# gnn-tracking/gnn_tracking

Hardware: AMD Instinct MI355X
Metric: edges_per_sec_fwd_bwd (higher is better)
Workload: dtype bf16

## Files before the change

gnn_tracking_amd/csrc/graph_index.hip:

```cpp
#include "host_util.h"
#include "tile_bf16.h"

namespace gnntrk {

constexpr int kTpb = 256;

constexpr int kSH = 8;
constexpr int kBins = 1 << kSH;
constexpr int kSortTpb = 512;
constexpr int kSortR = 10;
constexpr int kCap = kSortTpb * kSortR;
constexpr int kWin = 4096;
constexpr int kSplitTpb = 1024;
constexpr int kSplitWg = 1;
constexpr int kCountTpb = 1024;
constexpr int kSplitR = 4;
constexpr int kSplitTile = kSplitTpb * kSplitR;
constexpr int kMaxChunks = 512;
#ifndef GNNTRK_GI_HUB_BITMAP_MIN
#define GNNTRK_GI_HUB_BITMAP_MIN 65536
#endif
constexpr int64_t kMaxTable = (int64_t)96 << 20;
constexpr int kScanTpb = 256, kScanItems = 16, kScanTile = kScanTpb * kScanItems;

template <bool kNullable>
__device__ __forceinline__ int64_t gi_clamped(int64_t v, int64_t N, int *bad) {
    if (v < 0 || v >= N) {
        if (!kNullable || bad) atomicAdd(bad, 1);
        v = v < 0 ? 0 : N - 1;
    }
    return v;
}
__device__ __forceinline__ int4 gi_load4(const int32_t *a, int64_t e, int64_t e1) {
    if (e + 4 <= e1) return *reinterpret_cast<const int4 *>(a + e);
    return int4{e < e1 ? a[e] : 0, e + 1 < e1 ? a[e + 1] : 0, e + 2 < e1 ? a[e + 2] : 0, 0};
}

struct KeysCoo {
    const int64_t *src, *tgt;
    int64_t N;
    const uint8_t *label;
    const float *rows;
    int rows_stride;
    __device__ __forceinline__ uint32_t key(int64_t e, int *bad) const { return checked(tgt[e], bad); }
    int vec;
    const int32_t *rank;
    __device__ __forceinline__ uint32_t checked(int64_t v, int *bad) const {
        v = gi_clamped<true>(v, N, bad);
        return rank ? (uint32_t)rank[v] : (uint32_t)v;
    }
    __device__ __forceinline__ void keys4(int64_t e, int64_t e1, uint32_t k[4], int *bad) const {
        if (vec && e + 4 <= e1) {
            const longlong2 a = *reinterpret_cast<const longlong2 *>(tgt + e);
            const longlong2 b = *reinterpret_cast<const longlong2 *>(tgt + e + 2);
            k[0] = checked(a.x, bad);
            k[1] = checked(a.y, bad);
            k[2] = checked(b.x, bad);
            k[3] = checked(b.y, bad);
        } else {
#pragma unroll
            for (int q = 0; q < 4; ++q) k[q] = e + q < e1 ? key(e + q, bad) : 0u;
        }
    }
    struct Raw {
        longlong2 ta, tb, sa, sb;
        uint32_t l4;
    };
    __device__ __forceinline__ void load_raw(int64_t e, int64_t e1, Raw &r) const {
        if (vec && e + 4 <= e1) {
            r.ta = *reinterpret_cast<const longlong2 *>(tgt + e);
            r.tb = *reinterpret_cast<const longlong2 *>(tgt + e + 2);
            r.sa = *reinterpret_cast<const longlong2 *>(src + e);
            r.sb = *reinterpret_cast<const longlong2 *>(src + e + 2);
            r.l4 = label ? *reinterpret_cast<const uint32_t *>(label + e) : 0u;
        } else {
            long long t[4], u[4];
            r.l4 = 0u;
#pragma unroll
            for (int q = 0; q < 4; ++q) {
                const bool in = e + q < e1;
                t[q] = in ? tgt[e + q] : 0;
                u[q] = in ? src[e + q] : 0;
                if (in && label && label[e + q]) r.l4 |= 1u << (8 * q);
            }
            r.ta = longlong2{t[0], t[1]};
            r.tb = longlong2{t[2], t[3]};
            r.sa = longlong2{u[0], u[1]};
            r.sb = longlong2{u[2], u[3]};
        }
    }
    __device__ __forceinline__ void decode(const Raw &r, int64_t e, uint32_t k[4], uint32_t p[4], uint32_t v[4],
                                           int *bad) const {
        k[0] = checked(r.ta.x, nullptr);
        k[1] = checked(r.ta.y, nullptr);
        k[2] = checked(r.tb.x, nullptr);
        k[3] = checked(r.tb.y, nullptr);
        p[0] = checked(r.sa.x, bad);
        p[1] = checked(r.sa.y, bad);
        p[2] = checked(r.sb.x, bad);
        p[3] = checked(r.sb.y, bad);
#pragma unroll
        for (int q = 0; q < 4; ++q) v[q] = (uint32_t)(e + q) | (((r.l4 >> (8 * q)) & 0xffu) ? 0x80000000u : 0u);
    }
    __device__ __forceinline__ f32x4 row_raw(int64_t e) const {
        return *reinterpret_cast<const f32x4 *>(rows + e * rows_stride);
    }
};
struct KeysCoo32 {
    const int32_t *src, *tgt;
    const uint8_t *label;
    const float *rows;
    int rows_stride;
    int vec;
    __device__ __forceinline__ uint32_t key(int64_t e, int *) const { return (uint32_t)tgt[e]; }
    struct Raw {
        int4 t, s;
        uint32_t l4;
    };
    __device__ __forceinline__ void load_raw(int64_t e, int64_t e1, Raw &r) const {
        if (e + 4 <= e1) {
            r.t = *reinterpret_cast<const int4 *>(tgt + e);
            r.s = *reinterpret_cast<const int4 *>(src + e);
            if (!label) {
                r.l4 = 0u;
            } else if (vec) {
                r.l4 = *reinterpret_cast<const uint32_t *>(label + e);
            } else {
                r.l4 = (label[e] ? 1u : 0u) | (label[e + 1] ? 0x100u : 0u) | (label[e + 2] ? 0x10000u : 0u) |
                       (label[e + 3] ? 0x1000000u : 0u);
            }
        } else {
            int t[4], u[4];
            r.l4 = 0u;
#pragma unroll
            for (int q = 0; q < 4; ++q) {
                const bool in = e + q < e1;
                t[q] = in ? tgt[e + q] : 0;
                u[q] = in ? src[e + q] : 0;
                if (in && label && label[e + q]) r.l4 |= 1u << (8 * q);
            }
            r.t = int4{t[0], t[1], t[2], t[3]};
            r.s = int4{u[0], u[1], u[2], u[3]};
        }
    }
    __device__ __forceinline__ void decode(const Raw &r, int64_t e, uint32_t k[4], uint32_t p[4], uint32_t v[4],
                                           int *) const {
        k[0] = (uint32_t)r.t.x;
        k[1] = (uint32_t)r.t.y;
        k[2] = (uint32_t)r.t.z;
        k[3] = (uint32_t)r.t.w;
        p[0] = (uint32_t)r.s.x;
        p[1] = (uint32_t)r.s.y;
        p[2] = (uint32_t)r.s.z;
        p[3] = (uint32_t)r.s.w;
#pragma unroll
        for (int q = 0; q < 4; ++q) v[q] = (uint32_t)(e + q) | (((r.l4 >> (8 * q)) & 0xffu) ? 0x80000000u : 0u);
    }
    __device__ __forceinline__ f32x4 row_raw(int64_t e) const {
        return *reinterpret_cast<const f32x4 *>(rows + e * rows_stride);
    }
};
__device__ __forceinline__ void gi_remap4(const int64_t *__restrict__ src, const int64_t *__restrict__ tgt, int64_t e,
                                          int64_t e1, int64_t N, const int32_t *__restrict__ rank, int vec,
                                          int32_t *__restrict__ src32, int32_t *__restrict__ tgt32,
                                          int *__restrict__ bad, uint32_t kt[4]) {
    if (vec && e + 4 <= e1) {
        typedef int i4_hw __attribute__((ext_vector_type(4)));
        auto ld2 = [](const int64_t *p, long long &a, long long &b) {
            const i4_hw v = __builtin_nontemporal_load(reinterpret_cast<const i4_hw *>(p));
            a = (long long)(((unsigned long long)(uint32_t)v[1] << 32) | (uint32_t)v[0]);
            b = (long long)(((unsigned long long)(uint32_t)v[3] << 32) | (uint32_t)v[2]);
        };
        long long it[4], is[4];
        ld2(tgt + e, it[0], it[1]);
        ld2(tgt + e + 2, it[2], it[3]);
        ld2(src + e, is[0], is[1]);
        ld2(src + e + 2, is[2], is[3]);
#pragma unroll
        for (int q = 0; q < 4; ++q) {
            it[q] = gi_clamped<false>(it[q], N, bad);
            is[q] = gi_clamped<false>(is[q], N, bad);
        }
        const i4_hw ot = {rank[it[0]], rank[it[1]], rank[it[2]], rank[it[3]]};
        const i4_hw os = {rank[is[0]], rank[is[1]], rank[is[2]], rank[is[3]]};
        __builtin_nontemporal_store(ot, reinterpret_cast<i4_hw *>(tgt32 + e));
        __builtin_nontemporal_store(os, reinterpret_cast<i4_hw *>(src32 + e));
#pragma unroll
        for (int q = 0; q < 4; ++q) kt[q] = (uint32_t)ot[q];
    } else {
#pragma unroll
        for (int q = 0; q < 4; ++q) {
            kt[q] = 0u;
            if (e + q < e1) {
                const int t = rank[gi_clamped<false>(tgt[e + q], N, bad)], u = rank[gi_clamped<false>(src[e + q], N, bad)];
                tgt32[e + q] = t;
                src32[e + q] = u;
                kt[q] = (uint32_t)t;
            }
        }
    }
}
struct KeysCsr {
    const int32_t *src;
    __device__ __forceinline__ uint32_t key(int64_t e, int *) const { return (uint32_t)src[e]; }
    __device__ __forceinline__ void keys4(int64_t e, int64_t e1, uint32_t k[4], int *) const {
        const int4 a = gi_load4(src, e, e1);
        k[0] = (uint32_t)a.x;
        k[1] = (uint32_t)a.y;
        k[2] = (uint32_t)a.z;
        k[3] = (uint32_t)a.w;
    }
    struct Raw {
        int4 a;
    };
    __device__ __forceinline__ void load_raw(int64_t e, int64_t e1, Raw &r) const { r.a = gi_load4(src, e, e1); }
    __device__ __forceinline__ void decode(const Raw &r, int64_t e, uint32_t k[4], uint32_t p[4], uint32_t v[4],
                                           int *) const {
        k[0] = (uint32_t)r.a.x;
        k[1] = (uint32_t)r.a.y;
        k[2] = (uint32_t)r.a.z;
        k[3] = (uint32_t)r.a.w;
#pragma unroll
        for (int q = 0; q < 4; ++q) {
            p[q] = 0u;
            v[q] = (uint32_t)(e + q);
        }
    }
    __device__ __forceinline__ f32x4 row_raw(int64_t) const { return f32x4{0.f, 0.f, 0.f, 0.f}; }
};

__device__ __forceinline__ int gi_window_start(uint32_t first_key) {
    const int b = (int)(first_key >> kSH) - kWin / 3;
    return b < 0 ? 0 : b;
}

constexpr int kXcd = 8;
__device__ __forceinline__ int gi_chunk_of_block() {
    return (int)(blockIdx.x % kXcd) * (int)(gridDim.x / kXcd) + (int)(blockIdx.x / kXcd);
}
static int gi_chunk_grid(int n_chunks) { return (n_chunks + kXcd - 1) / kXcd * kXcd; }

__device__ __forceinline__ void gi_count4(const uint32_t k4[4], int64_t e, int64_t e1, int w0, uint32_t *s_cnt,
                                          uint32_t *__restrict__ tbl, int n_chunks, int c) {
    auto bump = [&](uint32_t b, uint32_t by) {
        const uint32_t d = b - (uint32_t)w0;
        if (d < (uint32_t)kWin)
            atomicAdd(&s_cnt[d], by);
        else
            atomicAdd(&tbl[(size_t)b * n_chunks + c], by);
    };
    uint32_t run_b = k4[0] >> kSH, run_n = 1;
#pragma unroll
    for (int q = 1; q < 4; ++q) {
        if (e + q >= e1) break;
        const uint32_t b = k4[q] >> kSH;
        if (b == run_b) {
            run_n += 1;
        } else {
            bump(run_b, run_n);
            run_b = b;
            run_n = 1;
        }
    }
    bump(run_b, run_n);
}
template <int TPB>
__device__ __forceinline__ void gi_count_flush(const uint32_t *s_cnt, int *s_lo, int *s_hi, int w0, int n_chunks, int c,
                                               uint32_t *__restrict__ tbl, int2 *__restrict__ range) {
    const int tid = threadIdx.x;
    __syncthreads();
    int lo = kWin, hi = -1;
    for (int d = tid; d < kWin; d += TPB) {
        const uint32_t v = s_cnt[d];
        if (v) {
            tbl[(size_t)(w0 + d) * n_chunks + c] = v;
            lo = d < lo ? d : lo;
            hi = d > hi ? d : hi;
        }
    }
    if (hi >= 0) {
        atomicMin(s_lo, lo);
        atomicMax(s_hi, hi);
    }
    __syncthreads();
    if (tid == 0) range[c] = int2{*s_lo, *s_hi};
}
template <class K>
__global__ __launch_bounds__(kCountTpb) void gi_count_kernel(K keys, int64_t E, int chunk, int n_chunks, int NB,
                                                             uint32_t *__restrict__ tbl, int2 *__restrict__ range,
                                                             int *__restrict__ bad) {
    __shared__ uint32_t s_cnt[kWin];
    __shared__ int s_lo, s_hi;
    const int tid = threadIdx.x, c = blockIdx.x;
    const int64_t e0 = (int64_t)c * chunk, e1 = e0 + chunk < E ? e0 + chunk : E;
    for (int d = tid; d < kWin; d += kCountTpb) s_cnt[d] = 0;
    if (tid == 0) {
        s_lo = kWin;
        s_hi = -1;
    }
    __syncthreads();
    const int w0 = gi_window_start(keys.key(e0, nullptr));
    for (int64_t e = e0 + 4 * tid; e < e1; e += 4 * kCountTpb) {
        uint32_t k4[4];
        keys.keys4(e, e1, k4, bad);
        gi_count4(k4, e, e1, w0, s_cnt, tbl, n_chunks, c);
    }
    gi_count_flush<kCountTpb>(s_cnt, &s_lo, &s_hi, w0, n_chunks, c, tbl, range);
    (void)NB;
}
constexpr int kRemapTpb = 1024;
__global__ __launch_bounds__(kRemapTpb, 8) void gi_remap_count_kernel(
    const int64_t *__restrict__ src, const int64_t *__restrict__ tgt, int64_t E, int64_t N,
    const int32_t *__restrict__ rank, int vec, int32_t *__restrict__ src32, int32_t *__restrict__ tgt32, int chunk,
    int n_chunks, uint32_t *__restrict__ tbl, int2 *__restrict__ range, int *__restrict__ bad) {
    __shared__ uint32_t s_cnt[kWin];
    __shared__ int s_lo, s_hi, s_w0;
    const int tid = threadIdx.x, c = gi_chunk_of_block();
    if (c >= n_chunks) return;
    const int64_t e0 = (int64_t)c * chunk, e1 = e0 + chunk < E ? e0 + chunk : E;
    for (int d = tid; d < kWin; d += kRemapTpb) s_cnt[d] = 0;
    if (tid == 0) {
        s_lo = kWin;
        s_hi = -1;
        s_w0 = gi_window_start((uint32_t)rank[gi_clamped<true>(tgt[e0], N, nullptr)]);
    }
    __syncthreads();
    const int w0 = s_w0;
    for (int64_t e = e0 + 4 * tid; e < e1; e += 4 * kRemapTpb) {
        uint32_t k4[4];
        gi_remap4(src, tgt, e, e1, N, rank, vec, src32, tgt32, bad, k4);
        gi_count4(k4, e, e1, w0, s_cnt, tbl, n_chunks, c);
    }
    gi_count_flush<kRemapTpb>(s_cnt, &s_lo, &s_hi, w0, n_chunks, c, tbl, range);
}

__global__ __launch_bounds__(kScanTpb) void gi_scan_sums_kernel(const uint32_t *__restrict__ v, int64_t n,
                                                                uint32_t *__restrict__ sums) {
    __shared__ uint32_t s[kScanTpb];
    const int tid = threadIdx.x;
    const int64_t i0 = (int64_t)blockIdx.x * kScanTile + (int64_t)tid * kScanItems;
    uint32_t t = 0;
    if (i0 + kScanItems <= n) {
#pragma unroll
        for (int q = 0; q < kScanItems / 4; ++q) {
            const uint4 a = *reinterpret_cast<const uint4 *>(v + i0 + 4 * q);
            t += a.x + a.y + a.z + a.w;
        }
    } else {
        for (int q = 0; q < kScanItems; ++q) t += i0 + q < n ? v[i0 + q] : 0u;
    }
    s[tid] = t;
    __syncthreads();
    for (int d = kScanTpb / 2; d > 0; d >>= 1) {
        if (tid < d) s[tid] += s[tid + d];
        __syncthreads();
    }
    if (tid == 0) sums[blockIdx.x] = s[0];
}

__global__ __launch_bounds__(kScanTpb) void gi_scan_apply_kernel(uint32_t *__restrict__ v, int64_t n,
                                                                 const uint32_t *__restrict__ sums, int n_chunks,
                                                                 uint32_t *__restrict__ base) {
    __shared__ uint32_t s[kScanTpb];
    __shared__ uint32_t s_before[kScanTpb / 64];
    const int tid = threadIdx.x;
    const int64_t i0 = (int64_t)blockIdx.x * kScanTile + (int64_t)tid * kScanItems;
    uint32_t before = 0;
    for (int i = tid; i < (int)blockIdx.x; i += kScanTpb) before += sums[i];
    for (int o = 32; o > 0; o >>= 1) before += (uint32_t)__shfl_xor((int)before, o);
    if ((tid & 63) == 0) s_before[tid >> 6] = before;
    uint32_t x[kScanItems];
    const bool full = i0 + kScanItems <= n;
    if (full) {
#pragma unroll
        for (int q = 0; q < kScanItems / 4; ++q) {
            const uint4 a = *reinterpret_cast<const uint4 *>(v + i0 + 4 * q);
            x[4 * q] = a.x;
            x[4 * q + 1] = a.y;
            x[4 * q + 2] = a.z;
            x[4 * q + 3] = a.w;
        }
    } else {
#pragma unroll
        for (int q = 0; q < kScanItems; ++q) x[q] = i0 + q < n ? v[i0 + q] : 0u;
    }
    uint32_t t = 0;
#pragma unroll
    for (int q = 0; q < kScanItems; ++q) t += x[q];
    s[tid] = t;
    __syncthreads();
    before = 0;
#pragma unroll
    for (int w = 0; w < kScanTpb / 64; ++w) before += s_before[w];
    for (int d = 1; d < kScanTpb; d <<= 1) {
        const uint32_t u = tid >= d ? s[tid - d] : 0u;
        __syncthreads();
        s[tid] += u;
        __syncthreads();
    }
    uint32_t run = before + s[tid] - t;
    int64_t bk = (i0 + n_chunks - 1) / n_chunks;
    int64_t nb = bk * n_chunks - i0;
#pragma unroll
    for (int q = 0; q < kScanItems; ++q) {
        const uint32_t c = x[q];
        x[q] = run;
        run += c;
        if (q == nb && i0 + q < n) {
            base[bk] = x[q];
            bk += 1;
            nb += n_chunks;
        }
    }
    if (full) {
#pragma unroll
        for (int q = 0; q < kScanItems / 4; ++q)
            *reinterpret_cast<uint4 *>(v + i0 + 4 * q) = uint4{x[4 * q], x[4 * q + 1], x[4 * q + 2], x[4 * q + 3]};
    } else {
#pragma unroll
        for (int q = 0; q < kScanItems; ++q)
            if (i0 + q < n) v[i0 + q] = x[q];
    }
}

__device__ __forceinline__ uint32_t gi_block_exscan(uint32_t v, uint32_t *s_wsum, uint32_t *total) {
    const int tid = threadIdx.x, lane = tid & 63, wv = tid >> 6;
    uint32_t inc = v;
#pragma unroll
    for (int d = 1; d < 64; d <<= 1) {
        const uint32_t o = __shfl(inc, lane - d);
        if (lane >= d) inc += o;
    }
    if (lane == 63) s_wsum[wv] = inc;
    __syncthreads();
    uint32_t pre = 0, tot = 0;
#pragma unroll
    for (int w = 0; w < kSplitTpb / 64; ++w) {
        const uint32_t t = s_wsum[w];
        pre += w < wv ? t : 0u;
        tot += t;
    }
    __syncthreads();
    *total = tot;
    return pre + inc - v;
}

template <bool ROWS>
struct GiRec {
    typedef uint2 type;
    static __device__ __forceinline__ uint2 make(uint32_t x, uint32_t y, const f32x4 &) { return uint2{x, y}; }
};
template <>
struct GiRec<true> {
    typedef uint4 type;
    static __device__ __forceinline__ uint4 make(uint32_t x, uint32_t y, const f32x4 &rv) {
        return uint4{x, y, bf16x2_pack(rv[0], rv[1]), bf16x2_pack(rv[2], rv[3])};
    }
};
template <class K, bool ROWS>
__global__ __launch_bounds__(kSplitTpb, kSplitWg * kSplitTpb / 256) void gi_split_kernel(K keys, int64_t E, int chunk, int n_chunks, int pbits,
                                                             uint32_t *__restrict__ tbl,
                                                             const int2 *__restrict__ range,
                                                             typename GiRec<ROWS>::type *__restrict__ part,
                                                             int *__restrict__ bad) {
    typedef typename GiRec<ROWS>::type Rec;
    __shared__ uint32_t s_off[kWin];
    __shared__ uint32_t s_cnt[kWin];
    __shared__ Rec s_stage[kSplitTile];
    __shared__ uint16_t s_slot[kSplitTile];
    __shared__ uint32_t s_wsum[kSplitTpb / 64];
    const int tid = threadIdx.x, c = blockIdx.x;
    const int64_t e0 = (int64_t)c * chunk, e1 = e0 + chunk < E ? e0 + chunk : E;
    const int w0 = gi_window_start(keys.key(e0, nullptr));
    const int2 r = range[c];
    const int n_r = r.y >= r.x ? r.y - r.x + 1 : 0;
    const int per = (n_r + kSplitTpb - 1) / kSplitTpb;
    for (int d = r.x + tid; d <= r.y; d += kSplitTpb) {
        s_off[d] = tbl[(size_t)(w0 + d) * n_chunks + c];
        s_cnt[d] = 0;
    }
    __syncthreads();
    static_assert(kSplitR == 4, "a lane takes four consecutive edges of a tile");
    typename K::Raw nraw;
    keys.load_raw(e0 + 4 * tid, e1, nraw);
    for (int64_t t0 = e0; t0 < e1; t0 += kSplitTile) {
        uint2 rec[kSplitR];
        f32x4 rraw[ROWS ? kSplitR : 1];
        uint32_t slot[kSplitR], rk[kSplitR];
        const int64_t et = t0 + 4 * tid;
        {
            uint32_t nk[kSplitR], np[kSplitR], nv[kSplitR];
            keys.decode(nraw, et, nk, np, nv, bad);
            keys.load_raw(et + kSplitTile, e1, nraw);
#pragma unroll
            for (int q = 0; q < kSplitR; ++q) {
                const int64_t e = et + q;
                slot[q] = 0xffffffffu;
                if (ROWS) rraw[q] = e < e1 ? keys.row_raw(e) : f32x4{0.f, 0.f, 0.f, 0.f};
                if (e < e1) {
                    const uint32_t v = nk[q], pl = np[q];
                    const uint32_t b = v >> kSH, low = v & (kBins - 1);
                    const uint32_t d = b - (uint32_t)w0;
                    rec[q] = uint2{nv[q], (low << pbits) | pl};
                    if (d < (uint32_t)kWin) {
                        slot[q] = d;
                        rk[q] = atomicAdd(&s_cnt[d], 1u);
                    } else {
                        const uint32_t pos = atomicAdd(&tbl[(size_t)b * n_chunks + c], 1u);
                        part[pos] = GiRec<ROWS>::make(rec[q].x, rec[q].y, rraw[ROWS ? q : 0]);
                    }
                }
            }
        }
        __syncthreads();
        const int d0 = r.x + tid * per;
        uint32_t mine = 0;
#pragma unroll 1
        for (int i = 0; i < per; ++i)
            if (d0 + i <= r.y) mine += s_cnt[d0 + i];
        uint32_t tile_n;
        uint32_t run = gi_block_exscan(mine, s_wsum, &tile_n);
#pragma unroll 1
        for (int i = 0; i < per; ++i)
            if (d0 + i <= r.y) {
                const uint32_t cn = s_cnt[d0 + i];
                s_cnt[d0 + i] = run;
                run += cn;
            }
        __syncthreads();
#pragma unroll
        for (int q = 0; q < kSplitR; ++q)
            if (slot[q] != 0xffffffffu) {
                const uint32_t spq = s_cnt[slot[q]] + rk[q];
                s_stage[spq] = GiRec<ROWS>::make(rec[q].x, rec[q].y, rraw[ROWS ? q : 0]);
                s_slot[spq] = (uint16_t)slot[q];
            }
        __syncthreads();
        for (uint32_t j = tid; j < tile_n; j += kSplitTpb) {
            const uint32_t d = s_slot[j];
            part[s_off[d] - s_cnt[d] + j] = s_stage[j];
        }
        __syncthreads();
#pragma unroll 1
        for (int i = 0; i < per; ++i)
            if (d0 + i <= r.y) {
                const int d = d0 + i;
                s_off[d] += (d == r.y ? tile_n : s_cnt[d + 1]) - s_cnt[d];
            }
        __syncthreads();
#pragma unroll 1
        for (int i = 0; i < per; ++i)
            if (d0 + i <= r.y) s_cnt[d0 + i] = 0;
        __syncthreads();
    }
}

template <bool ROWS>
struct OutCsr {
    static constexpr uint32_t kValMask = 0x7fffffffu;
    static constexpr bool kRows = ROWS;
    int32_t *perm, *tgt, *src, *rowptr;
    uint32_t pmask;
    uint8_t *label_csr;
    uint16_t *rows_csr;
    int rows_out_stride;
    __device__ __forceinline__ void ranked(uint32_t k, uint32_t val, uint32_t hi) const {
        perm[k] = (int32_t)(val & kValMask);
        src[k] = (int32_t)(hi & pmask);
        if (label_csr) label_csr[k] = (uint8_t)(val >> 31);
    }
    __device__ __forceinline__ void row(uint32_t k, uint2 r) const {
        if (ROWS) *reinterpret_cast<uint2 *>(rows_csr + (size_t)k * rows_out_stride) = r;
    }
    __device__ __forceinline__ void slot(uint32_t k, uint32_t node) const { tgt[k] = (int32_t)node; }
    __device__ __forceinline__ void node_start(int64_t node, uint32_t pos) const { rowptr[node] = (int32_t)pos; }
};
struct OutSrc {
    static constexpr uint32_t kValMask = 0xffffffffu;
    static constexpr bool kRows = false;
    int32_t *spos, *spos_inv, *rowptr;
    __device__ __forceinline__ void ranked(uint32_t k, uint32_t val, uint32_t) const {
        spos[k] = (int32_t)val;
        if (spos_inv) spos_inv[val] = (int32_t)k;
    }
    __device__ __forceinline__ void row(uint32_t, uint2) const {}
    __device__ __forceinline__ void slot(uint32_t, uint32_t) const {}
    __device__ __forceinline__ void node_start(int64_t node, uint32_t pos) const { rowptr[node] = (int32_t)pos; }
};

template <class O>
constexpr uint32_t kGiRS = O::kRows ? 2 : 1;
template <class O>
constexpr uint32_t kGiCapG = O::kRows ? (uint32_t)kCap * 2 / 3 : (uint32_t)kCap;

template <class O>
__device__ __forceinline__ void gi_sort_fits(uint2 (&rec)[kSortR], const uint2 (&rrow)[O::kRows ? kSortR : 1],
                                             uint32_t (&ord)[kSortR], uint32_t base, uint32_t M, uint32_t node0,
                                             int pbits, const uint32_t *s_hist, const uint32_t *s_start, uint2 *s_rec,
                                             uint16_t *s_fin, const O &out) {
    constexpr uint32_t VM = O::kValMask;
    const int tid = threadIdx.x;
#pragma unroll
    for (int q = 0; q < kSortR; ++q)
        if (tid + q * kSortTpb < M) {
            const uint32_t sl = s_start[rec[q].y >> pbits] + ord[q];
            s_rec[sl] = rec[q];
            ord[q] = sl;
        }
    __syncthreads();
    uint32_t dst[kSortR];
#pragma unroll
    for (int q = 0; q < kSortR; ++q) {
        const uint32_t j = tid + q * kSortTpb;
        if (j < M) {
            const uint2 r = s_rec[j];
            const uint32_t low = r.y >> pbits, st = s_start[low], n = s_hist[low];
            uint32_t cnt = 0;
            for (uint32_t t = 0; t < n; ++t) cnt += (s_rec[st + t].x & VM) < (r.x & VM) ? 1u : 0u;
            rec[q] = r;
            dst[q] = st + cnt;
            if (O::kRows) s_fin[j] = (uint16_t)dst[q];
            out.slot(base + j, node0 + low);
        }
    }
    __syncthreads();
#pragma unroll
    for (int q = 0; q < kSortR; ++q)
        if (tid + q * kSortTpb < M) s_rec[dst[q]] = rec[q];
    __syncthreads();
    for (uint32_t j = tid; j < M; j += kSortTpb) {
        const uint2 r = s_rec[j];
        out.ranked(base + j, r.x, r.y);
    }
    if (O::kRows) {
        __syncthreads();
#pragma unroll
        for (int q = 0; q < kSortR; ++q)
            if (tid + q * kSortTpb < M) s_rec[s_fin[ord[q]]] = rrow[O::kRows ? q : 0];
        __syncthreads();
        for (uint32_t j = tid; j < M; j += kSortTpb) out.row(base + j, s_rec[j]);
    }
}

template <class O>
__device__ __forceinline__ void gi_sort_group(const uint2 *__restrict__ part, uint32_t base, uint32_t M, uint32_t node0,
                                              int pbits, int g0, int g1, const uint32_t *s_hist,
                                              const uint32_t *s_start, uint32_t *s_cur, uint2 *s_rec, const O &out) {
    constexpr uint32_t VM = O::kValMask, kRS = kGiRS<O>;
    const int tid = threadIdx.x;
    uint32_t *s_pos32 = reinterpret_cast<uint32_t *>(s_rec + kGiCapG<O>);
    const uint32_t st0 = s_start[g0], n_g = (g1 < kBins ? s_start[g1] : M) - st0;
    __syncthreads();
    if (tid < kBins) s_cur[tid] = 0;
    __syncthreads();
    for (uint32_t i = tid; i < M; i += kSortTpb) {
        const uint2 r = part[(size_t)i * kRS];
        const int low = (int)(r.y >> pbits);
        if (low >= g0 && low < g1) {
            const uint32_t sl = s_start[low] - st0 + atomicAdd(&s_cur[low], 1u);
            s_rec[sl] = r;
            if (O::kRows) s_pos32[sl] = i;
        }
    }
    __syncthreads();
    for (uint32_t j = tid; j < n_g; j += kSortTpb) {
        const uint2 r = s_rec[j];
        const uint32_t low = r.y >> pbits, st = s_start[low] - st0, n = s_hist[low];
        uint32_t cnt = 0;
        for (uint32_t t = 0; t < n; ++t) cnt += (s_rec[st + t].x & VM) < (r.x & VM) ? 1u : 0u;
        out.ranked(base + st0 + st + cnt, r.x, r.y);
        if (O::kRows) out.row(base + st0 + st + cnt, part[(size_t)s_pos32[j] * kRS + (kRS - 1)]);
        out.slot(base + st0 + j, node0 + low);
    }
}

template <class O>
__device__ __forceinline__ void gi_hub_runs(const uint2 *__restrict__ part, uint32_t M, int pbits, int chunk, int g0,
                                            uint32_t *h_all, uint32_t *h_hub) {
    constexpr uint32_t VM = O::kValMask, kRS = kGiRS<O>;
    const int tid = threadIdx.x;
    __syncthreads();
    for (int t = tid; t < 2 * kMaxChunks; t += kSortTpb) h_all[t] = 0u;
    __syncthreads();
    for (uint32_t i = tid; i < M; i += kSortTpb) {
        const uint2 r = part[(size_t)i * kRS];
        const uint32_t ck = (r.x & VM) / (uint32_t)chunk;
        atomicAdd(&h_all[ck], 1u);
        if ((int)(r.y >> pbits) == g0) atomicAdd(&h_hub[ck], 1u);
    }
    __syncthreads();
    if (tid == 0) {
        uint32_t a_ = 0, h_ = 0;
        for (int ck = 0; ck < kMaxChunks; ++ck) {
            const uint32_t va = h_all[ck], vh = h_hub[ck];
            h_all[ck] = a_;
            h_hub[ck] = h_;
            a_ += va;
            h_ += vh;
        }
    }
    __syncthreads();
}
template <class O>
__device__ __forceinline__ void gi_hub_walk(const uint2 *__restrict__ part, uint32_t pos0, uint32_t M, int pbits,
                                            int chunk, int g0, const uint32_t *h_all, const uint32_t *h_hub,
                                            const O &out) {
    constexpr uint32_t VM = O::kValMask, kRS = kGiRS<O>;
    for (uint32_t i = threadIdx.x; i < M; i += kSortTpb) {
        const uint2 r = part[(size_t)i * kRS];
        if ((int)(r.y >> pbits) != g0) continue;
        const uint32_t ck = (r.x & VM) / (uint32_t)chunk;
        const uint32_t r0 = h_all[ck], r1 = ck + 1 < (uint32_t)kMaxChunks ? h_all[ck + 1] : M;
        uint32_t cnt = h_hub[ck];
        for (uint32_t t = r0; t < r1; ++t) {
            const uint2 q = part[(size_t)t * kRS];
            cnt += ((int)(q.y >> pbits) == g0 && (q.x & VM) < (r.x & VM)) ? 1u : 0u;
        }
        out.ranked(pos0 + cnt, r.x, r.y);
        if (O::kRows) out.row(pos0 + cnt, part[(size_t)i * kRS + (kRS - 1)]);
    }
}
constexpr uint32_t kHubSpanW = 4096, kHubSpan = kHubSpanW * 32;
template <class O>
__device__ __forceinline__ void gi_hub_bitmaps(const uint2 *__restrict__ part, uint32_t pos0, uint32_t M, uint32_t n,
                                               int pbits, int chunk, int g0, const uint32_t *h_all,
                                               const uint32_t *h_hub, uint32_t *bm, uint32_t *pw, const O &out) {
    constexpr uint32_t VM = O::kValMask, kRS = kGiRS<O>, kSpanW = kHubSpanW, kSpan = kHubSpan;
    const int tid = threadIdx.x;
    for (int ck = 0; ck < kMaxChunks; ++ck) {
        const uint32_t r0 = h_all[ck], r1 = ck + 1 < kMaxChunks ? h_all[ck + 1] : M;
        const uint32_t hub_here = (ck + 1 < kMaxChunks ? h_hub[ck + 1] : n) - h_hub[ck];
        if (hub_here == 0u) continue;
        uint32_t before = h_hub[ck];
        for (uint32_t lo = (uint32_t)ck * (uint32_t)chunk, sub = 0; sub < (uint32_t)chunk; sub += kSpan, lo += kSpan) {
            __syncthreads();
            for (uint32_t w = tid; w < kSpanW; w += kSortTpb) bm[w] = 0u;
            __syncthreads();
            for (uint32_t t = r0 + tid; t < r1; t += kSortTpb) {
                const uint2 q = part[(size_t)t * kRS];
                const uint32_t d = (q.x & VM) - lo;
                if ((int)(q.y >> pbits) == g0 && d < kSpan) atomicOr(&bm[d >> 5], 1u << (d & 31u));
            }
            __syncthreads();
            uint32_t mine = 0;
            constexpr uint32_t kPer = kSpanW / kSortTpb;
            for (uint32_t j = 0; j < kPer; ++j) mine += (uint32_t)__popc(bm[tid * kPer + j]);
            uint32_t *ts = pw;
            ts[tid] = mine;
            __syncthreads();
            for (uint32_t off = 1; off < (uint32_t)kSortTpb; off <<= 1) {
                const uint32_t v = tid >= (int)off ? ts[tid - off] : 0u;
                __syncthreads();
                ts[tid] += v;
                __syncthreads();
            }
            const uint32_t excl = ts[tid] - mine, span_total = ts[kSortTpb - 1];
            __syncthreads();
            uint32_t run_ = excl;
            for (uint32_t j = 0; j < kPer; ++j) {
                const uint32_t w = tid * kPer + j, c_ = (uint32_t)__popc(bm[w]);
                pw[w] = run_;
                run_ += c_;
            }
            __syncthreads();
            for (uint32_t t = r0 + tid; t < r1; t += kSortTpb) {
                const uint2 q = part[(size_t)t * kRS];
                const uint32_t d = (q.x & VM) - lo;
                if ((int)(q.y >> pbits) == g0 && d < kSpan) {
                    const uint32_t w = d >> 5;
                    const uint32_t below = (uint32_t)__popc(bm[w] & ((1u << (d & 31u)) - 1u));
                    out.ranked(pos0 + before + pw[w] + below, q.x, q.y);
                    if (O::kRows) out.row(pos0 + before + pw[w] + below, part[(size_t)t * kRS + (kRS - 1)]);
                }
            }
            before += span_total;
        }
    }
}

template <class O>
__global__ __launch_bounds__(kSortTpb) void gi_bucket_sort_kernel(const typename GiRec<O::kRows>::type *__restrict__ part_,
                                                                  const uint32_t *__restrict__ base_arr, int NB,
                                                                  int64_t N, int64_t E, int pbits, int chunk, O out) {
    constexpr uint32_t kRS = kGiRS<O>;
    const uint2 *__restrict__ part = reinterpret_cast<const uint2 *>(part_);
    __shared__ uint32_t s_hist[kBins], s_start[kBins], s_wsum[kBins / 64], s_cur[kBins];
    __shared__ uint2 s_rec[kCap];
    __shared__ uint16_t s_fin[O::kRows ? kCap : 1];
    const int tid = threadIdx.x, b = blockIdx.x, lane = tid & 63, wv = tid >> 6;
    const uint32_t base = base_arr[b], M = base_arr[b + 1] - base;
    part += (size_t)base * kRS;
    const uint32_t node0 = (uint32_t)b << kSH;
    const bool fits = M <= (uint32_t)kCap;
    if (tid < kBins) s_hist[tid] = 0;
    __syncthreads();
    uint2 rec[kSortR], rrow[O::kRows ? kSortR : 1];
    uint32_t ord[kSortR];
    if (fits) {
#pragma unroll
        for (int q = 0; q < kSortR; ++q) {
            const uint32_t i = tid + q * kSortTpb;
            if constexpr (O::kRows) {
                const uint4 v = i < M ? part_[base + i] : uint4{0u, 0u, 0u, 0u};
                rec[q] = uint2{v.x, v.y};
                rrow[q] = uint2{v.z, v.w};
            } else {
                rec[q] = i < M ? part[i] : uint2{0u, 0u};
            }
        }
#pragma unroll
        for (int q = 0; q < kSortR; ++q)
            if (tid + q * kSortTpb < M) ord[q] = atomicAdd(&s_hist[rec[q].y >> pbits], 1u);
    } else {
        for (uint32_t i = tid; i < M; i += kSortTpb) atomicAdd(&s_hist[part[(size_t)i * kRS].y >> pbits], 1u);
    }
    __syncthreads();
    uint32_t inc = 0, cnt_mine = 0;
    if (tid < kBins) {
        cnt_mine = s_hist[tid];
        inc = cnt_mine;
#pragma unroll
        for (int d = 1; d < 64; d <<= 1) {
            const uint32_t o = __shfl(inc, lane - d);
            if (lane >= d) inc += o;
        }
        if (lane == 63) s_wsum[wv] = inc;
    }
    __syncthreads();
    if (tid < kBins) {
        uint32_t pre = 0;
#pragma unroll
        for (int w = 0; w < kBins / 64; ++w) pre += w < wv ? s_wsum[w] : 0u;
        const uint32_t st = pre + inc - cnt_mine;
        s_start[tid] = st;
        if ((int64_t)node0 + tid < N) out.node_start(node0 + tid, base + st);
    }
    if (b == NB - 1 && tid == 0) out.node_start(N, (uint32_t)E);
    __syncthreads();
    if (fits) {
        gi_sort_fits(rec, rrow, ord, base, M, node0, pbits, s_hist, s_start, s_rec, s_fin, out);
    } else {
        int g0 = 0;
        while (g0 < kBins) {
            const uint32_t st0 = s_start[g0];
            int g1 = g0;
            while (g1 < kBins && (g1 + 1 < kBins ? s_start[g1 + 1] : M) - st0 <= kGiCapG<O>) ++g1;
            if (g1 == g0) {
                const uint32_t n = s_hist[g0];
                uint32_t *h_all = reinterpret_cast<uint32_t *>(s_rec), *h_hub = h_all + kMaxChunks;
                uint32_t *bm = h_hub + kMaxChunks, *pw = bm + kHubSpanW;
                static_assert((2 * kMaxChunks + 2 * kHubSpanW) * sizeof(uint32_t) <= kCap * sizeof(uint2),
                              "hub scratch exceeds s_rec");
                gi_hub_runs<O>(part, M, pbits, chunk, g0, h_all, h_hub);
                if (n <= (uint32_t)GNNTRK_GI_HUB_BITMAP_MIN)
                    gi_hub_walk(part, base + st0, M, pbits, chunk, g0, h_all, h_hub, out);
                else
                    gi_hub_bitmaps(part, base + st0, M, n, pbits, chunk, g0, h_all, h_hub, bm, pw, out);
                for (uint32_t j = tid; j < n; j += kSortTpb) out.slot(base + st0 + j, node0 + (uint32_t)g0);
                __syncthreads();
                g0 += 1;
                continue;
            }
            gi_sort_group(part, base, M, node0, pbits, g0, g1, s_hist, s_start, s_cur, s_rec, out);
            g0 = g1;
        }
    }
}

constexpr size_t kHeader = 256;
struct OwnPlan {
    bool ok;
    bool dense;
    int NB, n_chunks, chunk, bitsN;
    int64_t T;
    int n_tiles;
    size_t off_range, off_base, off_tbl, off_sums, off_part, bytes;
};

static int bits_for(int64_t n) {
    int b = 1;
    while (b < 32 && ((int64_t)1 << b) < n) ++b;
    return b;
}

static OwnPlan own_plan(int64_t N, int64_t E, bool rows) {
    OwnPlan p{};
    p.ok = false;
    if (N < 1 || E < 1) return p;
    p.bitsN = bits_for(N > 1 ? N : 2);
    if (p.bitsN + kSH > 32) return p;
    p.NB = (int)ceil_div(N, kBins);
    int nc = (int)ceil_div(E, 16384);
    if (nc > kMaxChunks) nc = kMaxChunks;
    int64_t chunk = ceil_div(E, nc);
    chunk = ceil_div(chunk, 4) * 4;
    p.chunk = (int)chunk;
    p.n_chunks = (int)ceil_div(E, chunk);
    p.T = (int64_t)p.NB * p.n_chunks;
    if (p.T > kMaxTable) return p;
    p.dense = E / p.NB > kCap * 9 / 10;
    p.n_tiles = (int)ceil_div(p.T + 1, kScanTile);
    size_t o = kHeader;
    p.off_tbl = o;
    o += align_up((size_t)(p.T + 1) * 4, 256);
    p.off_range = o;
    o += align_up((size_t)p.n_chunks * sizeof(int2), 256);
    p.off_base = o;
    o += align_up((size_t)(p.NB + 1) * 4, 256);
    p.off_sums = o;
    o += align_up((size_t)p.n_tiles * 4, 256);
    p.off_part = o;
    o += align_up((size_t)E * (rows ? 16 : 8), 256);
    p.bytes = o;
    p.ok = true;
    return p;
}

static uint32_t *own_tbl(const OwnPlan &p, char *ws) { return reinterpret_cast<uint32_t *>(ws + p.off_tbl); }
static int2 *own_range(const OwnPlan &p, char *ws) { return reinterpret_cast<int2 *>(ws + p.off_range); }

static int own_zero(const OwnPlan &p, char *ws, size_t head, hipStream_t stream) {
    return check_hip(hipMemsetAsync(ws + p.off_tbl - head, 0, head + (size_t)(p.T + 1) * 4, stream),
                     "counting sort(memset)");
}

template <class K>
static void own_count(const OwnPlan &p, K keys, int64_t E, char *ws, int *bad, hipStream_t stream) {
    hipLaunchKernelGGL((gi_count_kernel<K>), dim3(p.n_chunks), dim3(kCountTpb), 0, stream, keys, E, p.chunk,
                       p.n_chunks, p.NB, own_tbl(p, ws), own_range(p, ws), bad);
}

template <class K, class O>
static void own_sort(const OwnPlan &p, K keys, O out, int pbits, int64_t N, int64_t E, char *ws, int *bad,
                     hipStream_t stream) {
    typedef typename GiRec<O::kRows>::type Rec;
    int2 *range = own_range(p, ws);
    uint32_t *tbl = own_tbl(p, ws);
    uint32_t *base = reinterpret_cast<uint32_t *>(ws + p.off_base);
    uint32_t *sums = reinterpret_cast<uint32_t *>(ws + p.off_sums);
    Rec *part = reinterpret_cast<Rec *>(ws + p.off_part);
    hipLaunchKernelGGL(gi_scan_sums_kernel, dim3(p.n_tiles), dim3(kScanTpb), 0, stream, tbl, p.T + 1, sums);
    hipLaunchKernelGGL(gi_scan_apply_kernel, dim3(p.n_tiles), dim3(kScanTpb), 0, stream, tbl, p.T + 1, sums,
                       p.n_chunks, base);
    hipLaunchKernelGGL((gi_split_kernel<K, O::kRows>), dim3(p.n_chunks), dim3(kSplitTpb), 0, stream, keys, E, p.chunk,
                       p.n_chunks, pbits, tbl, range, part, bad);
    hipLaunchKernelGGL((gi_bucket_sort_kernel<O>), dim3(p.NB), dim3(kSortTpb), 0, stream, part, base, p.NB, N, E,
                       pbits, p.chunk, out);
}

__device__ __forceinline__ uint32_t gi_checked(int64_t v, int64_t N, const int32_t *rank, int *bad) {
    v = gi_clamped<false>(v, N, bad);
    return rank ? (uint32_t)rank[v] : (uint32_t)v;
}
__global__ __launch_bounds__(kTpb) void gi_keys_kernel(const int64_t *__restrict__ ids, int64_t E,
                                                       int64_t N, const int32_t *__restrict__ rank,
                                                       uint32_t *__restrict__ keys,
                                                       uint32_t *__restrict__ vals,
                                                       int *__restrict__ bad) {
    for (int64_t e = (int64_t)blockIdx.x * kTpb + threadIdx.x; e < E;
         e += (int64_t)gridDim.x * kTpb) {
        keys[e] = gi_checked(ids[e], N, rank, bad);
        vals[e] = (uint32_t)e;
    }
}

__global__ __launch_bounds__(kTpb) void gi_gather_src_kernel(const int64_t *__restrict__ src,
                                                             const uint32_t *__restrict__ perm,
                                                             int64_t E, int64_t N, const int32_t *__restrict__ rank,
                                                             int32_t *__restrict__ src_s,
                                                             uint32_t *__restrict__ keys,
                                                             uint32_t *__restrict__ vals,
                                                             int *__restrict__ bad) {
    for (int64_t k = (int64_t)blockIdx.x * kTpb + threadIdx.x; k < E;
         k += (int64_t)gridDim.x * kTpb) {
        const uint32_t s = gi_checked(src[perm[k]], N, rank, bad);
        src_s[k] = (int32_t)s;
        keys[k] = s;
        vals[k] = (uint32_t)k;
    }
}

__global__ __launch_bounds__(kTpb) void gi_rowptr_kernel(const uint32_t *__restrict__ sorted,
                                                         int64_t E, int64_t N,
                                                         int32_t *__restrict__ rowptr) {
    for (int64_t k = (int64_t)blockIdx.x * kTpb + threadIdx.x; k <= E;
         k += (int64_t)gridDim.x * kTpb) {
        const int64_t prev = (k == 0) ? -1 : (int64_t)sorted[k - 1];
        const int64_t cur = (k == E) ? N : (int64_t)sorted[k];
        for (int64_t n = prev + 1; n <= cur && n <= N; ++n) rowptr[n] = (int32_t)k;
    }
}

__global__ __launch_bounds__(kTpb) void gi_invert_kernel(const int32_t *__restrict__ spos, int64_t E,
                                                         int32_t *__restrict__ inv) {
    for (int64_t k = (int64_t)blockIdx.x * kTpb + threadIdx.x; k < E; k += (int64_t)gridDim.x * kTpb)
        inv[spos[k]] = (int32_t)k;
}

static int stream_grid(int64_t n) {
    int64_t g = ceil_div(n, kTpb);
    const int64_t cap = (int64_t)cu_count() * 8;
    if (g > cap) g = cap;
    return (int)(g < 1 ? 1 : g);
}

static size_t library_ws_bytes(int64_t E) {
    const size_t arr = align_up((size_t)(E > 0 ? E : 1) * sizeof(uint32_t), 256);
    return 256  + 3 * arr + align_up(sort_pairs_temp_bytes(E), 256);
}

static size_t remap_arr_bytes(int64_t E) { return align_up((size_t)(E > 0 ? E : 1) * sizeof(int32_t), 256); }
static size_t graph_index_ws_bytes(int64_t N, int64_t E, int carry) {
    const size_t lib = library_ws_bytes(E);
    const OwnPlan p = own_plan(N, E, (carry & 1) != 0);
    const size_t own = p.ok ? align_up(p.bytes, 256) + ((carry & 2) ? 2 * remap_arr_bytes(E) : 0) : 0;
    return own > lib ? own : lib;
}

__global__ __launch_bounds__(kTpb) void gi_gather_label_kernel(const uint8_t *__restrict__ label,
                                                               const int32_t *__restrict__ perm, int64_t E,
                                                               uint8_t *__restrict__ out) {
    for (int64_t k = (int64_t)blockIdx.x * kTpb + threadIdx.x; k < E; k += (int64_t)gridDim.x * kTpb)
        out[k] = label[perm[k]] ? 1 : 0;
}

static int library_build(const int64_t *edge_index, const gnntrk_graph_index *o, char *p, int *bad, int64_t N,
                         int64_t E, const int32_t *rank, hipStream_t stream) {
    p += 256;
    const size_t arr = align_up((size_t)(E > 0 ? E : 1) * sizeof(uint32_t), 256);
    uint32_t *keys_a = reinterpret_cast<uint32_t *>(p);
    p += arr;
    uint32_t *vals_a = reinterpret_cast<uint32_t *>(p);
    p += arr;
    uint32_t *keys_b = reinterpret_cast<uint32_t *>(p);
    p += arr;
    void *temp = p;
    const size_t temp_bytes = sort_pairs_temp_bytes(E);
    const int bits = bits_for(N > 1 ? N : 2);
    const int grid = stream_grid(E + 1);
    const int64_t *src = edge_index, *tgt = edge_index + E;
    hipLaunchKernelGGL(gi_keys_kernel, dim3(grid), dim3(kTpb), 0, stream, tgt, E, N, rank, keys_a, vals_a, bad);
    uint32_t *tgt_sorted = reinterpret_cast<uint32_t *>(o->tgt);
    int rc = sort_pairs_u32(keys_a, tgt_sorted, vals_a, reinterpret_cast<uint32_t *>(o->perm), E, bits, temp,
                            temp_bytes, stream);
    if (rc) return rc;
    hipLaunchKernelGGL(gi_rowptr_kernel, dim3(grid), dim3(kTpb), 0, stream, tgt_sorted, E, N, o->rowptr_t);
    hipLaunchKernelGGL(gi_gather_src_kernel, dim3(grid), dim3(kTpb), 0, stream, src,
                       reinterpret_cast<const uint32_t *>(o->perm), E, N, rank, o->src, keys_a, vals_a, bad);
    rc = sort_pairs_u32(keys_a, keys_b, vals_a, reinterpret_cast<uint32_t *>(o->spos), E, bits, temp, temp_bytes,
                        stream);
    if (rc) return rc;
    hipLaunchKernelGGL(gi_rowptr_kernel, dim3(grid), dim3(kTpb), 0, stream, keys_b, E, N, o->rowptr_s);
    if (o->spos_inv)
        hipLaunchKernelGGL(gi_invert_kernel, dim3(grid), dim3(kTpb), 0, stream, o->spos, E, o->spos_inv);
    return GNNTRK_OK;
}

static int graph_index_build(const int64_t *edge_index, const gnntrk_graph_index *o,
                             const gnntrk_graph_index_carry *cy, void *ws, size_t ws_bytes, int flags,
                             hipStream_t stream) {
    if (!o) return fail(GNNTRK_EINVAL, "graph_index_build: NULL output descriptor");
    const int64_t E = o->n_edges, N = o->n_nodes;
    if (E < 0 || N < 0 || E > 0x7fffffff || N > 0x7fffffff)
        return fail(GNNTRK_EUNSUPPORTED, "graph_index_build: sizes must fit int32");
    if (!o->rowptr_t || !o->rowptr_s || (E > 0 && (!o->perm || !o->tgt || !o->src || !o->spos)))
        return fail(GNNTRK_EINVAL, "graph_index_build: NULL output array");
    if (E > 0 && !edge_index) return fail(GNNTRK_EINVAL, "graph_index_build: NULL edge_index");
    const uint8_t *label = cy ? cy->edge_label : nullptr;
    const float *rows = cy ? cy->edge_rows : nullptr;
    const int32_t *rank = cy ? cy->node_rank : nullptr;
    if (E > 0 && label && !cy->label_csr) return fail(GNNTRK_EINVAL, "graph_index_build: carried label without output");
    if (E > 0 && rows &&
        (!cy->rows_csr_bf16 || cy->rows_stride < 4 || cy->rows_stride % 4 != 0 || ((uintptr_t)rows & 15) != 0 ||
         cy->out_stride < 4 || cy->out_stride % 4 != 0 || ((uintptr_t)cy->rows_csr_bf16 & 7) != 0))
        return fail(GNNTRK_EINVAL,
                    "graph_index_build: carried rows must be 16-byte aligned fp32 [E, 4] with a row stride that is a "
                    "multiple of 4 floats; the bf16 output 8-byte aligned with a stride that is a multiple of 4");
    if (!ws || ws_bytes < graph_index_ws_bytes(N, E, (rows ? 1 : 0) | (rank ? 2 : 0)))
        return fail(GNNTRK_EINVAL, "graph_index_build: workspace too small");

    char *p = reinterpret_cast<char *>(ws);
    int *bad = reinterpret_cast<int *>(p);
    int rc = GNNTRK_OK;
    const OwnPlan plan = own_plan(N, E, rows != nullptr);
    const bool own = E > 0 && plan.ok && !(flags & 1) && (!plan.dense || (flags & 2));
    if (!own) {
        rc = check_hip(hipMemsetAsync(bad, 0, kHeader, stream), "graph_index_build(memset)");
        if (rc) return rc;
    }
    if (E > 0) {
        if (own) {
            const int vec = (((uintptr_t)edge_index | (uintptr_t)(edge_index + E)) & 15) == 0 &&
                            (!label || ((uintptr_t)label & 3) == 0);
            const KeysCoo k1{edge_index, edge_index + E, N, label, rows, rows ? cy->rows_stride : 0, vec, nullptr};
            const uint32_t pmask = (uint32_t)(((uint64_t)1 << plan.bitsN) - 1);
            const OutCsr<true> o1r{o->perm, o->tgt, o->src, o->rowptr_t, pmask, label ? cy->label_csr : nullptr,
                                   rows ? cy->rows_csr_bf16 : nullptr, rows ? cy->out_stride : 0};
            const OutCsr<false> o1{o->perm, o->tgt, o->src, o->rowptr_t, pmask, label ? cy->label_csr : nullptr,
                                   nullptr, 0};
            auto first_sort = [&](auto keys) {
                if (rows)
                    own_sort(plan, keys, o1r, plan.bitsN, N, E, p, bad, stream);
                else
                    own_sort(plan, keys, o1, plan.bitsN, N, E, p, bad, stream);
            };
            rc = own_zero(plan, p, kHeader, stream);
            if (rc) return rc;
            if (rank) {
                int32_t *src32 = reinterpret_cast<int32_t *>(p + align_up(plan.bytes, 256));
                int32_t *tgt32 = reinterpret_cast<int32_t *>(p + align_up(plan.bytes, 256) + remap_arr_bytes(E));
                const int vec_ids = (((uintptr_t)edge_index | (uintptr_t)(edge_index + E)) & 15) == 0;
                hipLaunchKernelGGL(gi_remap_count_kernel, dim3(gi_chunk_grid(plan.n_chunks)), dim3(kRemapTpb), 0, stream, edge_index,
                                   edge_index + E, E, N, rank, vec_ids, src32, tgt32, plan.chunk, plan.n_chunks,
                                   own_tbl(plan, p), own_range(plan, p), bad);
                first_sort(KeysCoo32{src32, tgt32, label, rows, rows ? cy->rows_stride : 0,
                                     (!label || ((uintptr_t)label & 3) == 0) ? 1 : 0});
            } else {
                own_count(plan, k1, E, p, bad, stream);
                first_sort(k1);
            }
            const KeysCsr k2{o->src};
            const OutSrc o2{o->spos, o->spos_inv, o->rowptr_s};
            rc = own_zero(plan, p, 0, stream);
            if (rc) return rc;
            own_count(plan, k2, E, p, bad, stream);
            own_sort(plan, k2, o2, 0, N, E, p, bad, stream);
        } else {
            rc = library_build(edge_index, o, p, bad, N, E, rank, stream);
            if (rc) return rc;
            if (label)
                hipLaunchKernelGGL(gi_gather_label_kernel, dim3(stream_grid(E)), dim3(kTpb), 0, stream, label, o->perm, E,
                                   cy->label_csr);
            if (rows)
                rc = rows_to_bf16_launch(rows, 4, cy->rows_stride, o->perm, E, cy->rows_csr_bf16, cy->out_stride, stream);
        }
        if (rc) return rc;
    } else {
        rc = check_hip(hipMemsetAsync(o->rowptr_t, 0, (size_t)(N + 1) * 4, stream), "memset");
        if (rc) return rc;
        rc = check_hip(hipMemsetAsync(o->rowptr_s, 0, (size_t)(N + 1) * 4, stream), "memset");
        if (rc) return rc;
    }
    return check_launch("graph_index_build");
}

__global__ __launch_bounds__(kTpb) void gi_place_kernel(gnntrk_graph_index part, gnntrk_graph_index batch, int32_t noff,
                                                        int32_t eoff, const uint8_t *__restrict__ lab_in,
                                                        uint8_t *__restrict__ lab_out, const uint2 *__restrict__ rows_in,
                                                        uint2 *__restrict__ rows_out, const int32_t *__restrict__ nperm_in,
                                                        int32_t *__restrict__ nperm_out, const int32_t *__restrict__ nrank_in,
                                                        int32_t *__restrict__ nrank_out) {
    const int64_t E = part.n_edges, N = part.n_nodes;
    const int64_t n4 = (E + 3) / 4;
    const bool vec = ((eoff & 3) == 0);
    for (int64_t i = (int64_t)blockIdx.x * kTpb + threadIdx.x; i < n4; i += (int64_t)gridDim.x * kTpb) {
        const int64_t k = 4 * i;
        if (vec && k + 4 <= E) {
            auto mv = [&](const int32_t *src, int32_t *dst, int32_t add) {
                int4 v = *reinterpret_cast<const int4 *>(src + k);
                v.x += add;
                v.y += add;
                v.z += add;
                v.w += add;
                *reinterpret_cast<int4 *>(dst + eoff + k) = v;
            };
            mv(part.perm, batch.perm, eoff);
            mv(part.tgt, batch.tgt, noff);
            mv(part.src, batch.src, noff);
            mv(part.spos, batch.spos, eoff);
            if (part.spos_inv && batch.spos_inv) mv(part.spos_inv, batch.spos_inv, eoff);
            if (lab_in) *reinterpret_cast<uint32_t *>(lab_out + eoff + k) = *reinterpret_cast<const uint32_t *>(lab_in + k);
            if (rows_in) {
#pragma unroll
                for (int q = 0; q < 4; ++q) rows_out[eoff + k + q] = rows_in[k + q];
            }
        } else {
            for (int q = 0; q < 4 && k + q < E; ++q) {
                const int64_t j = k + q;
                batch.perm[eoff + j] = part.perm[j] + eoff;
                batch.tgt[eoff + j] = part.tgt[j] + noff;
                batch.src[eoff + j] = part.src[j] + noff;
                batch.spos[eoff + j] = part.spos[j] + eoff;
                if (part.spos_inv && batch.spos_inv) batch.spos_inv[eoff + j] = part.spos_inv[j] + eoff;
                if (lab_in) lab_out[eoff + j] = lab_in[j];
                if (rows_in) rows_out[eoff + j] = rows_in[j];
            }
        }
    }
    for (int64_t n = (int64_t)blockIdx.x * kTpb + threadIdx.x; n <= N; n += (int64_t)gridDim.x * kTpb) {
        batch.rowptr_t[noff + n] = part.rowptr_t[n] + eoff;
        batch.rowptr_s[noff + n] = part.rowptr_s[n] + eoff;
        if (n < N && nperm_in) {
            nperm_out[noff + n] = nperm_in[n] + noff;
            nrank_out[noff + n] = nrank_in[n] + noff;
        }
    }
}
__device__ __forceinline__ uint32_t no_image(float v) {
    const uint32_t u = __float_as_uint(v);
    return u ^ ((u >> 31) ? 0xffffffffu : 0x80000000u);
}
__device__ __forceinline__ float no_unimage(uint32_t u) {
    return __uint_as_float((u >> 31) ? (u ^ 0x80000000u) : ~u);
}
__global__ __launch_bounds__(kTpb) void no_keys_kernel(const float *__restrict__ key, int64_t stride,
                                                       const int64_t *__restrict__ batch, int64_t n,
                                                       unsigned long long *__restrict__ keys,
                                                       uint32_t *__restrict__ vals) {
    for (int64_t i = (int64_t)blockIdx.x * kTpb + threadIdx.x; i < n; i += (int64_t)gridDim.x * kTpb) {
        const uint32_t u = no_image(key[i * stride]);
        const unsigned long long b = batch ? (unsigned long long)(uint32_t)batch[i] : 0ull;
        keys[i] = (b << 32) | u;
        vals[i] = (uint32_t)i;
    }
}
__global__ __launch_bounds__(kTpb) void no_keys32_kernel(const float *__restrict__ key, int64_t stride,
                                                         const int64_t *__restrict__ batch, int64_t n, int ebits,
                                                         uint32_t *__restrict__ keys, uint32_t *__restrict__ vals) {
    for (int64_t i = (int64_t)blockIdx.x * kTpb + threadIdx.x; i < n; i += (int64_t)gridDim.x * kTpb) {
        const uint32_t u = no_image(key[i * stride]);
        const uint32_t b = (batch && ebits > 0) ? (uint32_t)batch[i] << (32 - ebits) : 0u;
        keys[i] = b | (ebits > 0 ? u >> ebits : u);
        vals[i] = (uint32_t)i;
    }
}
__global__ __launch_bounds__(kTpb) void no_finish_kernel(const uint32_t *__restrict__ sorted, int64_t n,
                                                         int32_t *__restrict__ perm, int32_t *__restrict__ rank) {
    for (int64_t i = (int64_t)blockIdx.x * kTpb + threadIdx.x; i < n; i += (int64_t)gridDim.x * kTpb) {
        const uint32_t v = sorted[i];
        perm[i] = (int32_t)v;
        rank[v] = (int32_t)i;
    }
}
constexpr int kNoLevels = 1 << 16;
constexpr int kNoMaxEvents = 64;
constexpr size_t kNoHead = 1024;
__global__ __launch_bounds__(kTpb) void no_minmax_kernel(const float *__restrict__ key, int64_t stride,
                                                         const int64_t *__restrict__ batch, int64_t n, int64_t n_events,
                                                         uint32_t *__restrict__ mm, float *__restrict__ keyc) {
    __shared__ uint32_t s_mm[2 * kNoMaxEvents];
    for (int t = threadIdx.x; t < 2 * kNoMaxEvents; t += kTpb) s_mm[t] = 0u;
    __syncthreads();
    for (int64_t i0 = (int64_t)blockIdx.x * kTpb; i0 < n; i0 += (int64_t)gridDim.x * kTpb) {
        const int64_t i = i0 + threadIdx.x;
        const bool in = i < n;
        const float v = in ? key[i * stride] : 0.f;
        if (in && keyc) keyc[i] = v;
        long long b = (in && batch) ? batch[i] : 0;
        b = b < 0 ? 0 : b >= n_events ? n_events - 1 : b;
        const uint32_t u = no_image(v);
        const bool on = in && v == v;
        uint32_t nlo = on ? ~u : 0u, hi = on ? u : 0u;
        const int b0 = __shfl((int)b, 0);
        if (__ballot(in && (int)b != b0) == 0ull) {
            for (int o = 32; o > 0; o >>= 1) {
                const uint32_t l2 = (uint32_t)__shfl_xor((int)nlo, o), h2 = (uint32_t)__shfl_xor((int)hi, o);
                nlo = l2 > nlo ? l2 : nlo;
                hi = h2 > hi ? h2 : hi;
            }
            if ((threadIdx.x & 63) == 0) {
                atomicMax(&s_mm[2 * b0], nlo);
                atomicMax(&s_mm[2 * b0 + 1], hi);
            }
        } else if (on) {
            atomicMax(&s_mm[2 * (int)b], nlo);
            atomicMax(&s_mm[2 * (int)b + 1], hi);
        }
    }
    __syncthreads();
    for (int t = threadIdx.x; t < 2 * kNoMaxEvents; t += kTpb)
        if (s_mm[t]) atomicMax(&mm[t], s_mm[t]);
}
__global__ __launch_bounds__(kTpb) void no_qkeys_kernel(const float *__restrict__ key, int64_t stride,
                                                        const int64_t *__restrict__ batch, int64_t n, int64_t n_events,
                                                        const uint32_t *__restrict__ mm, int32_t *__restrict__ q,
                                                        int *__restrict__ bad) {
    __shared__ float s_lo[kNoMaxEvents], s_scale[kNoMaxEvents];
    for (int t = threadIdx.x; t < kNoMaxEvents; t += kTpb) {
        const uint32_t ulo = ~mm[2 * t], uhi = mm[2 * t + 1];
        const bool any = t < n_events && ulo <= uhi;
        const float lo = any ? no_unimage(ulo) : 0.f, hi = any ? no_unimage(uhi) : 0.f;
        s_lo[t] = lo;
        s_scale[t] = hi > lo ? (float)(kNoLevels - 1) / (hi - lo) : 0.f;
    }
    __syncthreads();
    for (int64_t i = (int64_t)blockIdx.x * kTpb + threadIdx.x; i < n; i += (int64_t)gridDim.x * kTpb) {
        const float v = key[i * stride];
        long long b = batch ? batch[i] : 0;
        if (b < 0 || b >= n_events) {
            atomicAdd(bad, 1);
            b = b < 0 ? 0 : n_events - 1;
        }
        float t = (v - s_lo[b]) * s_scale[b];
        t = t < 0.f ? 0.f : t;
        const uint32_t lvl = (v != v || t >= (float)(kNoLevels - 1)) ? (uint32_t)(kNoLevels - 1) : (uint32_t)t;
        q[i] = (int32_t)((uint32_t)b * (uint32_t)kNoLevels + lvl);
    }
}
struct OutNode {
    static constexpr uint32_t kValMask = 0xffffffffu;
    static constexpr bool kRows = false;
    int32_t *perm, *rank;
    __device__ __forceinline__ void ranked(uint32_t k, uint32_t val, uint32_t) const {
        perm[k] = (int32_t)val;
        rank[val] = (int32_t)k;
    }
    __device__ __forceinline__ void row(uint32_t, uint2) const {}
    __device__ __forceinline__ void slot(uint32_t, uint32_t) const {}
    __device__ __forceinline__ void node_start(int64_t, uint32_t) const {}
};
constexpr int64_t kNoMaxKeys = (int64_t)kNoMaxEvents * kNoLevels;
static bool node_order_own(int64_t n, int64_t n_events, const int64_t *batch, OwnPlan &plan, int64_t &keys) {
    const int64_t ev = batch ? n_events : 1;
    if (ev < 1) return false;
    if (ev > kNoMaxEvents) return false;
    keys = ev * kNoLevels;
    if (keys > kNoMaxKeys) return false;
    plan = own_plan(keys, n, false);
    return plan.ok && !plan.dense;
}

}

using namespace gnntrk;

extern "C" {

size_t gnntrk_graph_index_workspace_bytes(int64_t n_nodes, int64_t n_edges) {
    return graph_index_ws_bytes(n_nodes, n_edges, 0);
}

size_t gnntrk_graph_index_workspace_bytes_carry(int64_t n_nodes, int64_t n_edges, int32_t carry_rows) {
    return graph_index_ws_bytes(n_nodes, n_edges, carry_rows);
}

int gnntrk_graph_index_build(const int64_t *edge_index, const gnntrk_graph_index *out, void *workspace,
                             size_t workspace_bytes, void *stream) {
    return graph_index_build(edge_index, out, nullptr, workspace, workspace_bytes, 0, (hipStream_t)stream);
}

int gnntrk_graph_index_build_ex(const int64_t *edge_index, const gnntrk_graph_index *out, void *workspace,
                                size_t workspace_bytes, int32_t flags, void *stream) {
    return graph_index_build(edge_index, out, nullptr, workspace, workspace_bytes, flags, (hipStream_t)stream);
}

int gnntrk_graph_index_build_carry(const int64_t *edge_index, const gnntrk_graph_index *out,
                                   const gnntrk_graph_index_carry *carry, void *workspace, size_t workspace_bytes,
                                   int32_t flags, void *stream) {
    return graph_index_build(edge_index, out, carry, workspace, workspace_bytes, flags, (hipStream_t)stream);
}

int gnntrk_graph_index_place(const gnntrk_graph_index *part, int64_t node_offset, int64_t edge_offset,
                             const gnntrk_graph_index *batch, const uint8_t *label_part, uint8_t *label_batch,
                             const uint16_t *rows_part, uint16_t *rows_batch, const int32_t *node_perm_part,
                             int32_t *node_perm_batch, const int32_t *node_rank_part, int32_t *node_rank_batch,
                             void *stream_) {
    hipStream_t stream = (hipStream_t)stream_;
    if (!part || !batch) return fail(GNNTRK_EINVAL, "graph_index_place: NULL descriptor");
    if (node_offset < 0 || edge_offset < 0 || node_offset + part->n_nodes > batch->n_nodes ||
        edge_offset + part->n_edges > batch->n_edges || batch->n_edges > 0x7fffffff || batch->n_nodes > 0x7fffffff)
        return fail(GNNTRK_EINVAL, "graph_index_place: the event does not fit the batch at these offsets");
    if ((label_part != nullptr) != (label_batch != nullptr) || (rows_part != nullptr) != (rows_batch != nullptr) ||
        (node_perm_part != nullptr) != (node_perm_batch != nullptr) || (node_perm_part != nullptr) != (node_rank_part != nullptr) ||
        (node_rank_part != nullptr) != (node_rank_batch != nullptr))
        return fail(GNNTRK_EINVAL, "graph_index_place: carried / node-order arrays must come in pairs");
    if (rows_part && ((((uintptr_t)rows_part | (uintptr_t)rows_batch) & 7) != 0))
        return fail(GNNTRK_EINVAL, "graph_index_place: carried rows are 8-byte rows");
    const int64_t work = part->n_edges / 4 > part->n_nodes ? part->n_edges / 4 : part->n_nodes;
    hipLaunchKernelGGL(gi_place_kernel, dim3(stream_grid(work + 1)), dim3(kTpb), 0, stream, *part, *batch,
                       (int32_t)node_offset, (int32_t)edge_offset, label_part, label_batch,
                       reinterpret_cast<const uint2 *>(rows_part), reinterpret_cast<uint2 *>(rows_batch), node_perm_part,
                       node_perm_batch, node_rank_part, node_rank_batch);
    return check_launch("graph_index_place");
}

size_t gnntrk_node_order_workspace_bytes(int64_t n_nodes) {
    const size_t m = (size_t)(n_nodes > 0 ? n_nodes : 1);
    const size_t t64 = sort_pairs_u64_temp_bytes(n_nodes), t32 = sort_pairs_temp_bytes(n_nodes);
    const size_t lib = 2 * align_up(m * 8, 256) + 2 * align_up(m * 4, 256) + align_up(t64 > t32 ? t64 : t32, 256);
    const OwnPlan p = own_plan(kNoMaxKeys, n_nodes > 0 ? n_nodes : 1, false);
    const size_t own = kNoHead + (p.ok ? align_up(p.bytes, 256) : 0) + 2 * align_up(m * 4, 256);
    return lib > own ? lib : own;
}

int gnntrk_node_order(const float *key, int64_t key_stride, const int64_t *batch, int64_t n_events, int64_t n_nodes,
                      int32_t *perm, int32_t *rank, void *workspace, size_t workspace_bytes, void *stream_) {
    hipStream_t stream = (hipStream_t)stream_;
    if (n_nodes < 0 || n_nodes > 0x7fffffff) return fail(GNNTRK_EUNSUPPORTED, "node_order: sizes must fit int32");
    if (n_nodes == 0) return GNNTRK_OK;
    if (!key || key_stride < 1 || !perm || !rank) return fail(GNNTRK_EINVAL, "node_order: NULL argument");
    if (!workspace || workspace_bytes < gnntrk_node_order_workspace_bytes(n_nodes))
        return fail(GNNTRK_EINVAL, "node_order: workspace too small");
    char *p = reinterpret_cast<char *>(workspace);
    const int grid = stream_grid(n_nodes);
    OwnPlan plan;
    int64_t n_keys = 0;
    if (node_order_own(n_nodes, n_events, batch, plan, n_keys)) {
        static_assert((2 * kNoMaxEvents + 1) * sizeof(uint32_t) <= kNoHead - kHeader, "the head block holds the minima / maxima and the flag word");
        uint32_t *mm = reinterpret_cast<uint32_t *>(p);
        int *bad = reinterpret_cast<int *>(mm + 2 * kNoMaxEvents);
        char *sort_ws = p + kNoHead - kHeader;
        const size_t arr = align_up((size_t)n_nodes * 4, 256);
        int32_t *q = reinterpret_cast<int32_t *>(p + kNoHead + align_up(plan.bytes, 256));
        float *keyc = reinterpret_cast<float *>(reinterpret_cast<char *>(q) + arr);
        const int rc = own_zero(plan, sort_ws, kNoHead, stream);
        if (rc) return rc;
        const int64_t ev = batch ? n_events : 1;
        hipLaunchKernelGGL(no_minmax_kernel, dim3(grid), dim3(kTpb), 0, stream, key, key_stride, batch, n_nodes, ev,
                           mm, keyc);
        hipLaunchKernelGGL(no_qkeys_kernel, dim3(grid), dim3(kTpb), 0, stream, keyc, (int64_t)1, batch, n_nodes, ev, mm,
                           q, bad);
        const KeysCsr keys{q};
        own_count(plan, keys, n_nodes, sort_ws, bad, stream);
        own_sort(plan, keys, OutNode{perm, rank}, 0, n_keys, n_nodes, sort_ws, bad, stream);
        return check_launch("node_order");
    }
    const size_t k8 = align_up((size_t)n_nodes * 8, 256), v4 = align_up((size_t)n_nodes * 4, 256);
    unsigned long long *ka = reinterpret_cast<unsigned long long *>(p), *kb = reinterpret_cast<unsigned long long *>(p + k8);
    uint32_t *va = reinterpret_cast<uint32_t *>(p + 2 * k8), *vb = reinterpret_cast<uint32_t *>(p + 2 * k8 + v4);
    void *temp = p + 2 * k8 + 2 * v4;
    int ebits = batch ? 32 : 0;
    if (batch && n_events > 0) {
        ebits = 0;
        while (ebits < 32 && ((int64_t)1 << ebits) < n_events) ++ebits;
    }
    int rc;
    if (ebits <= 8) {
        uint32_t *k32a = reinterpret_cast<uint32_t *>(ka), *k32b = reinterpret_cast<uint32_t *>(kb);
        hipLaunchKernelGGL(no_keys32_kernel, dim3(grid), dim3(kTpb), 0, stream, key, key_stride, batch, n_nodes, ebits,
                           k32a, va);
        rc = sort_pairs_u32(k32a, k32b, va, vb, n_nodes, 32, temp, sort_pairs_temp_bytes(n_nodes), stream);
    } else {
        hipLaunchKernelGGL(no_keys_kernel, dim3(grid), dim3(kTpb), 0, stream, key, key_stride, batch, n_nodes, ka, va);
        rc = sort_pairs_u64_bits(ka, kb, va, vb, n_nodes, 32 + ebits, temp, sort_pairs_u64_temp_bytes(n_nodes), stream);
    }
    if (rc) return rc;
    hipLaunchKernelGGL(no_finish_kernel, dim3(grid), dim3(kTpb), 0, stream, vb, n_nodes, perm, rank);
    return check_launch("node_order");
}

}
```

gnn_tracking_amd/edge_classifier.py:

```python

from __future__ import annotations

import math

import torch
from torch import Tensor, nn

from . import _capi, locality, ops, ops_bf16, precision
from .edge_order import EdgeOrdered, NodeOrdered
from .hparams import HyperparametersMixin, assert_feat_dim
from .mlp import MLP
from .resin import ResIN


def _n_events(data) -> int:
    ptr = getattr(data, "ptr", None)
    return int(ptr.numel()) - 1 if isinstance(ptr, Tensor) and ptr.numel() > 1 else 0


class ECForGraphTCN(nn.Module, HyperparametersMixin):
    def __init__(self, *, node_indim: int, edge_indim: int, interaction_node_dim: int = 5,
                 interaction_edge_dim: int = 4, hidden_dim: int | float | None = None,
                 L_ec: int = 3, alpha: float = 0.5, residual_type="skip1",
                 use_intermediate_edge_embeddings: bool = True, use_node_embedding: bool = True,
                 residual_kwargs: dict | None = None):
        super().__init__()
        self.save_hyperparameters()
        residual_kwargs = dict(residual_kwargs or {})
        residual_kwargs["collect_hidden_edge_embeds"] = use_intermediate_edge_embeddings
        self.relu = nn.ReLU()
        self.ec_node_encoder = MLP(node_indim, interaction_node_dim, hidden_dim=hidden_dim, L=2,
                                   bias=False)
        self.ec_edge_encoder = MLP(edge_indim, interaction_edge_dim, hidden_dim=hidden_dim, L=2,
                                   bias=False)
        self.ec_resin = ResIN(node_dim=interaction_node_dim, edge_dim=interaction_edge_dim,
                              object_hidden_dim=hidden_dim, relational_hidden_dim=hidden_dim,
                              alpha=alpha, n_layers=L_ec, residual_type=residual_type,
                              residual_kwargs=residual_kwargs)
        w_input_dim = interaction_edge_dim
        if use_intermediate_edge_embeddings:
            w_input_dim = self.ec_resin.concat_edge_embeddings_length
        if use_node_embedding:
            w_input_dim += interaction_node_dim * 2
        self.W = MLP(input_size=w_input_dim, output_size=1, hidden_dim=hidden_dim, L=3)
        self.latent_dim = (interaction_node_dim, interaction_edge_dim)

    def forward(self, data) -> dict[str, Tensor]:
        x, edge_index, edge_attr = data.x, data.edge_index, data.edge_attr
        assert_feat_dim(x, self.hparams.node_indim)
        assert_feat_dim(edge_attr, self.hparams.edge_indim)
        bf16 = precision.use_bf16()
        y = getattr(data, "y", None)
        col = locality.order_column(data)
        batch = getattr(data, "batch", None)
        gi = ops.placed_graph_index(edge_index, x.shape[0])
        if gi is None:
            gi = ops.graph_index(edge_index, x.shape[0],
                                 carry_label=y if isinstance(y, Tensor) and self.training else None,
                                 carry_rows=edge_attr if bf16 and edge_attr.shape[1] == 4 else None,
                                 order_by=None if col is None else (x, col, batch if isinstance(batch, Tensor) else None,
                                                                    _n_events(data)))
        E = gi.n_edges
        nperm = gi.node_perm

        if bf16:
            h = self.ec_node_encoder.fused([ops.Seg(ops_bf16.to_rows16(x, nperm))], epilogue=_capi.EPI_RELU)
            ea_csr = ops.carried_rows(gi, edge_attr)
            if ea_csr is None:
                ea_csr = ops_bf16.to_rows16(edge_attr, gi.perm)
            e = self.ec_edge_encoder.fused([ops.Seg(ea_csr)], n_rows=E, epilogue=_capi.EPI_RELU)
        else:
            h = self.ec_node_encoder.fused([ops.Seg(x) if nperm is None else ops.Seg(x, nperm, False, "perm")],
                                           n_rows=x.shape[0], epilogue=_capi.EPI_RELU)
            e = self.ec_edge_encoder.fused([ops.Seg(edge_attr, gi.perm, False, "perm")],
                                           n_rows=E, epilogue=_capi.EPI_RELU)
        h, e, es = self.ec_resin.forward_csr(gi, h, e)

        segs = []
        if self.hparams.use_node_embedding:
            segs += [ops.Seg(h, gi.src, False, ("src", gi)), ops.Seg(h, gi.tgt, False, ("tgt", gi))]
        if self.hparams.use_intermediate_edge_embeddings:
            segs += [ops.Seg(ops_bf16.grad_tap(t) if i + 1 < len(es) else t) for i, t in enumerate(es)]
        else:
            segs.append(ops.Seg(e))
        eps = 0.001
        def head():
            return self.W.fused(segs, n_rows=E, epilogue=_capi.EPI_SIGMOID, ca=eps, cb=1 - 2 * eps).squeeze()

        w = None
        if bf16 and self.training:
            lin = self.W.linears()
            w = ops.deferred_head(segs, [m.weight for m in lin], [m.bias for m in lin], gi, y, n_rows=E,
                                  ca=eps, cb=1 - 2 * eps, head=head)
        return {
            "W": w if w is not None else EdgeOrdered(head(), gi),
            "node_embedding": h if nperm is None else NodeOrdered(h, gi),
            "edge_embedding": EdgeOrdered(e, gi),
        }


class PerfectEdgeClassification(nn.Module, HyperparametersMixin):
    def __init__(self, tpr=1.0, tnr=1.0, false_below_pt=0.0):
        super().__init__()
        self.save_hyperparameters()
        assert 0.0 <= tpr <= 1.0
        assert 0.0 <= tnr <= 1.0
        self.tpr, self.tnr, self.false_below_pt = tpr, tnr, false_below_pt

    def forward(self, data) -> dict[str, Tensor]:
        truth = data.y.bool()
        w = truth
        exact = lambda p: math.isclose(p, 1.0, rel_tol=1e-5, abs_tol=1e-8)
        none = torch.zeros_like(truth)
        if not exact(self.tpr):
            kept = torch.rand(int(truth.sum()), device=truth.device) <= self.tpr
            w = none.masked_scatter(truth, kept)
        if not exact(self.tnr):
            negative = ~w
            promoted = torch.rand(int(negative.sum()), device=truth.device) > self.tnr
            w = w | none.masked_scatter(negative, promoted)
        if self.false_below_pt > 0.0:
            w = w.masked_fill(data.pt < self.false_below_pt, False)
        return {"W": w.to(torch.float32)}
```

gnn_tracking_amd/ops.py:

```python

from __future__ import annotations

import os

import collections
import ctypes as C
import contextlib
import dataclasses
import weakref
from typing import Optional, Sequence

import torch
from torch import Tensor

from . import _capi

__all__ = [
    "GraphIndex", "graph_index", "Seg", "fused_mlp", "segment_sum", "permute_rows",
    "axpby", "bce_loss", "knn_graph", "edge_labels", "edge_features",
]


def _stream(t: Tensor):
    if t.is_cuda:
        return torch.cuda.current_stream(t.device).cuda_stream
    return None


def _p(t: Optional[Tensor]):
    return None if t is None else t.data_ptr()


def _as_rows(t: Tensor) -> Tensor:
    if t.dim() == 1:
        t = t.unsqueeze(1)
    if t.dim() != 2:
        raise ValueError(f"expected a 1-D or 2-D tensor, got shape {tuple(t.shape)}")
    if t.dtype != torch.float32:
        raise TypeError(f"gnn_tracking_amd kernels are fp32; got {t.dtype}")
    if t.shape[1] > 1 and t.stride(1) != 1:
        t = t.contiguous()
    if t.shape[0] > 1 and t.stride(0) < t.shape[1]:
        t = t.contiguous()
    return t


def _row_stride(t: Tensor) -> int:
    return t.stride(0) if t.shape[0] > 1 else max(t.shape[1], 1)


def _ws(nbytes: int, like: Tensor) -> Tensor:
    return torch.empty(max(int(nbytes), 16), dtype=torch.uint8, device=like.device)


class KernelTimer:

    def __init__(self):
        self.records = []

    def summary(self) -> dict:
        out: dict = {}
        for key, e0, e1, fl, by, rows in self.records:
            d = out.setdefault(key, dict(launches=0, ms=0.0, flops=0.0, bytes=0.0, rows=0))
            d["launches"] += 1
            d["ms"] += e0.elapsed_time(e1)
            d["flops"] += fl
            d["bytes"] += by
            d["rows"] += rows
        return out


_TIMER: Optional[KernelTimer] = None

_EVENT_POOL: list = []


def reserve_timing_events(n: int) -> None:
    while len(_EVENT_POOL) < n:
        e = torch.cuda.Event(enable_timing=True)
        e.record()
        e.record()
        _EVENT_POOL.append(e)


def timing_event():
    return _EVENT_POOL.pop() if _EVENT_POOL else torch.cuda.Event(enable_timing=True)


def set_kernel_timer(t: Optional[KernelTimer]) -> None:
    global _TIMER
    _TIMER = t


def kernel_key(lib, args, backward: bool, bf16: bool = False) -> str:
    if _TIMER is None:
        return ""
    buf = C.create_string_buffer(160)
    _capi.check(lib.gnntrk_mlp_kernel_name(C.byref(args.mlp), args.n_seg, args.seg,
                                           (1 if backward else 0) + (2 if bf16 else 0), buf,
                                           len(buf)), lib)
    return buf.value.decode()


def _mlp_flops_per_row(m) -> int:
    mid = m.hidden * m.hidden if m.n_layers == 3 else 0
    return 2 * (m.in_dim * m.hidden + mid + m.hidden * m.out_dim)


class _timed:
    def __init__(self, t: Tensor, key: str, flops: float, nbytes: float, rows: int):
        self.on = _TIMER is not None and t.is_cuda
        self.args = (key, flops, nbytes, rows)

    def __enter__(self):
        if self.on:
            self.e0 = timing_event()
            self.e1 = timing_event()
            self.e0.record()

    def __exit__(self, *exc):
        if self.on:
            self.e1.record()
            key, fl, by, rows = self.args
            _TIMER.records.append((key, self.e0, self.e1, fl, by, rows))


@dataclasses.dataclass
class GraphIndex:

    n_nodes: int
    n_edges: int
    perm: Tensor
    tgt: Tensor
    src: Tensor
    rowptr_t: Tensor
    rowptr_s: Tensor
    spos: Tensor
    spos_inv: Tensor
    ready: object = None
    node_perm: Optional[Tensor] = None
    node_rank: Optional[Tensor] = None
    order_sig: object = None
    placed: bool = False

    def node_values(self, t: Tensor) -> Tensor:
        return t if self.node_perm is None else t.index_select(0, self.node_perm)


_GI_CACHE: dict[int, tuple] = {}


def clear_graph_index_cache() -> None:
    _GI_CACHE.clear()


_VALIDATE = bool(os.environ.get("GNNTRK_VALIDATE"))
_GI_FLAGS = int(os.environ.get("GNNTRK_GI_FLAGS", "0"))
CARRY = os.environ.get("GNNTRK_GI_CARRY", "1") != "0"


def node_order(x: Tensor, col: int, batch: Optional[Tensor] = None, n_events: int = 0):
    _capi.require_device(x)
    if x.dtype != torch.float32 or x.dim() != 2:
        raise TypeError("node_order: x must be fp32 [N, F]")
    if x.stride(1) != 1 or x.stride(0) < x.shape[1]:
        x = x.contiguous()
    lib = _capi.load()
    n = int(x.shape[0])
    key = x[:, col]
    if batch is not None:
        if batch.dtype != torch.int64 or batch.numel() != n or batch.device != x.device:
            raise ValueError("node_order: batch must be int64 [N] on the device of x")
        batch = batch.contiguous()
    perm = torch.empty(n, dtype=torch.int32, device=x.device)
    rank = torch.empty(n, dtype=torch.int32, device=x.device)
    ws = _ws(lib.gnntrk_node_order_workspace_bytes(n), x)
    _capi.check(lib.gnntrk_node_order(_p(key), int(x.stride(0)), _p(batch), int(n_events), n, _p(perm), _p(rank), _p(ws), ws.numel(),
                                      _stream(x)), lib)
    return perm, rank


def _order_sig(order_by):
    if order_by is None:
        return None
    x, col, batch = order_by[:3]
    return (id(x), x._version, int(col), None if batch is None else (id(batch), batch._version))


def graph_index(edge_index: Tensor, n_nodes: int, *, cache: bool = True,
                validate: Optional[bool] = None, flags: Optional[int] = None,
                carry_label: Optional[Tensor] = None, carry_rows: Optional[Tensor] = None,
                order_by: Optional[tuple] = None) -> GraphIndex:
    if edge_index.dim() != 2 or edge_index.shape[0] != 2:
        raise ValueError(f"edge_index must be [2,E], got {tuple(edge_index.shape)}")
    if edge_index.dtype != torch.int64:
        raise TypeError("edge_index must be int64 (PyG convention)")
    _capi.require_device(edge_index)
    sig = _order_sig(order_by)
    key = (id(edge_index), sig is not None)
    if cache:
        hit = _GI_CACHE.get(key)
        if hit is not None:
            ref, ver, nn, gi = hit
            if (ref() is edge_index and ver == edge_index._version and nn == n_nodes and gi.order_sig == sig
                    and (sig is None or gi._order_ref() is order_by[0])):
                return _join(gi)
    lib = _capi.load()
    ei = edge_index.contiguous()
    E = int(ei.shape[1])
    dev = ei.device
    mk = lambda n: torch.empty(n, dtype=torch.int32, device=dev)
    gi = GraphIndex(n_nodes, E, mk(E), mk(E), mk(E), mk(n_nodes + 1), mk(n_nodes + 1), mk(E), mk(E))
    d = _capi.GraphIndex(n_nodes, E, _p(gi.perm), _p(gi.tgt), _p(gi.src), _p(gi.rowptr_t),
                         _p(gi.rowptr_s), _p(gi.spos), _p(gi.spos_inv))
    cy = _capi.GraphIndexCarry()
    if order_by is not None:
        if int(order_by[0].shape[0]) != n_nodes:
            raise ValueError("graph_index(order_by): x must hold one row per node")
        gi.node_perm, gi.node_rank = node_order(*order_by)
        gi.order_sig, gi._order_ref = sig, weakref.ref(order_by[0])
        cy.node_rank = _p(gi.node_rank)
    lab = rows = None
    if CARRY and carry_label is not None and E > 0 and _carry_label_ok(carry_label, E, dev):
        lab = carry_label.detach().view(torch.uint8).contiguous().view(-1)
        lab_csr = torch.empty(E, dtype=torch.uint8, device=dev)
        cy.edge_label, cy.label_csr = _p(lab), _p(lab_csr)
    if CARRY and carry_rows is not None and E > 0 and _carry_rows_ok(carry_rows, E, dev):
        from . import ops_bf16
        rows = carry_rows.detach()
        rows_csr = ops_bf16.empty_rows(E, 4, dev)
        cy.edge_rows, cy.rows_csr_bf16 = _p(rows), _p(rows_csr)
        cy.rows_stride, cy.out_stride = int(rows.stride(0)), int(rows_csr.stride(0))
    ws = _ws(lib.gnntrk_graph_index_workspace_bytes_carry(n_nodes, E, int(rows is not None) | (2 if gi.node_rank is not None else 0)), ei)
    _capi.check(lib.gnntrk_graph_index_build_carry(_p(ei), C.byref(d), C.byref(cy), _p(ws), ws.numel(),
                                                   _GI_FLAGS if flags is None else int(flags), _stream(ei)), lib)
    if lab is not None:
        gi._label_csr = (id(carry_label), carry_label._version, weakref.ref(carry_label), lab_csr)
    if rows is not None:
        gi._rows_csr = (id(carry_rows), carry_rows._version, weakref.ref(carry_rows), rows_csr)
    if _VALIDATE if validate is None else validate:
        bad = int(ws[:4].view(torch.int32).item())
        if bad:
            raise IndexError(f"edge_index: {bad} node ids out of range [0, {n_nodes})")
    gi._built_from = (weakref.ref(edge_index), edge_index._version)
    if cache:
        _cache_put(edge_index, n_nodes, gi)
    return gi


def place_graph_indices(parts: Sequence[GraphIndex], batch, order_col: Optional[int] = None) -> GraphIndex:
    parts = list(parts)
    if not parts:
        raise ValueError("place_graph_indices: no parts")
    ei = batch.edge_index
    _capi.require_device(ei)
    lib = _capi.load()
    dev = ei.device
    N, E = sum(p.n_nodes for p in parts), sum(p.n_edges for p in parts)
    if int(batch.x.shape[0]) != N or int(ei.shape[1]) != E:
        raise ValueError(f"place_graph_indices: the parts hold {N} nodes / {E} edges, the batch {batch.x.shape[0]} / {ei.shape[1]}")
    mk = lambda n: torch.empty(n, dtype=torch.int32, device=dev)
    gi = GraphIndex(N, E, mk(E), mk(E), mk(E), mk(N + 1), mk(N + 1), mk(E), mk(E))
    ordered = [p.node_perm is not None for p in parts]
    lab = [getattr(p, "_label_csr", None) for p in parts]
    rows = [getattr(p, "_rows_csr", None) for p in parts]
    full = [i for i, p in enumerate(parts) if p.n_edges > 0]
    has_lab = bool(full) and lab[full[0]] is not None
    has_rows = bool(full) and rows[full[0]] is not None
    if any((lab[i] is not None) != has_lab or (rows[i] is not None) != has_rows for i in full):
        raise ValueError("place_graph_indices: the parts must agree in their carried inputs")
    ptr = getattr(batch, "ptr", None)
    if isinstance(ptr, Tensor) and ptr.numel() == len(parts) + 1 and not ptr.is_cuda:
        sizes = (ptr[1:] - ptr[:-1]).tolist()
        if sizes != [p.n_nodes for p in parts]:
            raise ValueError(f"place_graph_indices: the events of the batch hold {sizes} nodes, the parts {[p.n_nodes for p in parts]}")
    want_order = any(ordered) or order_col is not None
    ident = {}
    if want_order and not all(ordered):
        for i, p in enumerate(parts):
            if not ordered[i]:
                ident[i] = torch.arange(p.n_nodes, dtype=torch.int32, device=dev)
    if want_order:
        gi.node_perm, gi.node_rank = mk(N), mk(N)
    lab_b = torch.empty(E, dtype=torch.uint8, device=dev) if has_lab else None
    rows_b = None
    if has_rows:
        from . import ops_bf16
        rows_b = ops_bf16.empty_rows(E, 4, dev)
    d = _capi.GraphIndex(N, E, _p(gi.perm), _p(gi.tgt), _p(gi.src), _p(gi.rowptr_t), _p(gi.rowptr_s), _p(gi.spos),
                         _p(gi.spos_inv))
    no = eo = 0
    st = _stream(ei)
    for i, (p, l, r) in enumerate(zip(parts, lab, rows)):
        dp = _capi.GraphIndex(p.n_nodes, p.n_edges, _p(p.perm), _p(p.tgt), _p(p.src), _p(p.rowptr_t), _p(p.rowptr_s),
                              _p(p.spos), _p(p.spos_inv))
        pperm, prank = (ident[i], ident[i]) if i in ident else (p.node_perm, p.node_rank)
        _capi.check(lib.gnntrk_graph_index_place(
            C.byref(dp), no, eo, C.byref(d), _p(None if l is None else l[3]), _p(None if l is None else lab_b),
            _p(None if r is None else r[3]), _p(None if r is None else rows_b), _p(pperm), _p(gi.node_perm), _p(prank),
            _p(gi.node_rank), st), lib)
        no += p.n_nodes
        eo += p.n_edges
    y, ea = getattr(batch, "y", None), getattr(batch, "edge_attr", None)
    if lab_b is not None and isinstance(y, Tensor):
        gi._label_csr = (id(y), y._version, weakref.ref(y), lab_b)
    if rows_b is not None and isinstance(ea, Tensor):
        gi._rows_csr = (id(ea), ea._version, weakref.ref(ea), rows_b)
    if want_order:
        col = parts[ordered.index(True)].order_sig[2] if any(ordered) else int(order_col)
        bt = getattr(batch, "batch", None)
        gi.order_sig, gi._order_ref = _order_sig((batch.x, col, bt if isinstance(bt, Tensor) else None)), weakref.ref(batch.x)
    gi._built_from = (weakref.ref(ei), ei._version)
    gi.placed = True
    _cache_put(ei, N, gi)
    return gi


def placed_graph_index(edge_index: Tensor, n_nodes: int) -> Optional[GraphIndex]:
    for renumbered in (True, False):
        hit = _GI_CACHE.get((id(edge_index), renumbered))
        if hit is not None and hit[0]() is edge_index and hit[1] == edge_index._version and hit[2] == n_nodes and hit[3].placed:
            return _join(hit[3])
    return None


def _carry_label_ok(y: Tensor, E: int, dev) -> bool:
    return y.dtype in (torch.bool, torch.uint8) and y.numel() == E and y.device == dev


def _carry_rows_ok(r: Tensor, E: int, dev) -> bool:
    return (r.device == dev and r.dtype == torch.float32 and r.dim() == 2 and tuple(r.shape) == (E, 4) and r.stride(1) == 1
            and r.stride(0) >= 4 and r.stride(0) % 4 == 0 and r.data_ptr() % 16 == 0)


def _carried(gi: GraphIndex, slot: str, t: Tensor):
    hit = getattr(gi, slot, None)
    if hit is not None and hit[0] == id(t) and hit[1] == t._version and hit[2]() is t:
        return hit[3]
    return None


def carried_label(gi: GraphIndex, y: Tensor):
    return _carried(gi, "_label_csr", y)


def carried_rows(gi: GraphIndex, rows: Tensor):
    return _carried(gi, "_rows_csr", rows)


_GI_CACHE_MAX = 4


def _cache_put(edge_index: Tensor, n_nodes: int, gi: GraphIndex) -> None:
    for k in [k for k, v in _GI_CACHE.items() if v[0]() is None]:
        _GI_CACHE.pop(k, None)
    while len(_GI_CACHE) >= _GI_CACHE_MAX:
        _GI_CACHE.pop(next(iter(_GI_CACHE)))
    _GI_CACHE[(id(edge_index), gi.order_sig is not None)] = (weakref.ref(edge_index), edge_index._version, n_nodes, gi)


def _join(gi: GraphIndex) -> GraphIndex:
    if gi.ready is not None:
        cur = torch.cuda.current_stream(gi.perm.device)
        cur.wait_event(gi.ready)
        carried = [getattr(gi, slot)[3] for slot in ("_label_csr", "_rows_csr") if getattr(gi, slot, None) is not None]
        for t in (gi.perm, gi.tgt, gi.src, gi.rowptr_t, gi.rowptr_s, gi.spos, gi.spos_inv,
                  getattr(gi, "node_perm", None), getattr(gi, "node_rank", None), *carried):
            if isinstance(t, torch.Tensor) and t.is_cuda:
                t.record_stream(cur)
        gi.ready = None
    return gi


def prefetch_graph_index(edge_index: Tensor, n_nodes: int, stream, x: Optional[Tensor] = None,
                         batch: Optional[Tensor] = None) -> GraphIndex:
    from . import locality
    col = None if x is None else locality.key_column(x)
    with torch.cuda.stream(stream):
        gi = graph_index(edge_index, n_nodes, cache=False, order_by=None if col is None else (x, col, batch))
        gi.ready = torch.cuda.Event()
        gi.ready.record(stream)
    _cache_put(edge_index, n_nodes, gi)
    return gi


def _fold_of(by: str, gi):
    if by == "tgt":
        return gi.rowptr_t, None
    if by == "src":
        return gi.rowptr_s, gi.spos
    raise ValueError(by)


def _segment_sum_raw(rows: Tensor, rowptr: Tensor, pos: Optional[Tensor], n_seg: int,
                     out: Optional[Tensor] = None, accumulate: bool = False) -> Tensor:
    lib = _capi.load()
    rows = _as_rows(rows)
    dim = rows.shape[1]
    if out is None:
        out = torch.empty(n_seg, dim, dtype=torch.float32, device=rows.device)
        accumulate = False
    _capi.check(lib.gnntrk_segment_sum(_p(rows), dim, _row_stride(rows), _p(rowptr), _p(pos),
                                       n_seg, _p(out), _row_stride(out), int(accumulate),
                                       _stream(rows)), lib)
    return out


def _permute_raw(x: Tensor, idx: Tensor, scatter: bool) -> Tensor:
    lib = _capi.load()
    x2 = _as_rows(x)
    m = int(idx.shape[0])
    if scatter and m != x2.shape[0]:
        raise ValueError("permute_rows(scatter): idx must be a permutation of the rows")
    out = torch.empty(m, x2.shape[1], dtype=torch.float32, device=x2.device)
    _capi.check(lib.gnntrk_permute_rows(_p(x2), x2.shape[1], _row_stride(x2), _p(idx), m,
                                        _p(out), _row_stride(out), int(scatter),
                                        _stream(x2)), lib)
    return out.view(-1) if x.dim() == 1 else out


def _axpby_raw(a: float, x: Tensor, b: float = 0.0, y: Optional[Tensor] = None,
               relu_mask: Optional[Tensor] = None) -> Tensor:
    lib = _capi.load()
    x = x.contiguous()
    y = None if y is None else y.contiguous()
    relu_mask = None if relu_mask is None else relu_mask.contiguous()
    out = torch.empty_like(x)
    _capi.check(lib.gnntrk_axpby(a, _p(x), b, _p(y), _p(relu_mask), _p(out), x.numel(),
                                 _stream(x)), lib)
    return out


class _SegmentSum(torch.autograd.Function):
    @staticmethod
    def forward(ctx, rows, gi: GraphIndex, by: str):
        _capi.require_device(rows)
        ctx.gi, ctx.by = gi, by
        return _segment_sum_raw(rows, *_fold_of(by, gi), gi.n_nodes)

    @staticmethod
    def backward(ctx, g):
        gi = ctx.gi
        idx = gi.tgt if ctx.by == "tgt" else gi.src
        return _permute_raw(g.contiguous(), idx, scatter=False), None, None


def segment_sum(rows: Tensor, gi: GraphIndex, by: str = "tgt") -> Tensor:
    if rows.dtype == torch.bfloat16:
        if rows.dim() == 2 and rows.shape[1] > 16:
            return _SegmentSum.apply(rows.float(), gi, by).to(torch.bfloat16)
        from . import ops_bf16
        return ops_bf16.SegmentSum16.apply(rows, gi, by)
    return _SegmentSum.apply(rows, gi, by)


class _PermuteRows(torch.autograd.Function):
    @staticmethod
    def forward(ctx, x, idx, scatter: bool):
        _capi.require_device(x)
        ctx.idx, ctx.scatter = idx, scatter
        return _permute_raw(x, idx, scatter)

    @staticmethod
    def backward(ctx, g):
        return _permute_raw(g.contiguous(), ctx.idx, not ctx.scatter), None, None


def permute_rows(x: Tensor, idx: Tensor, scatter: bool = False) -> Tensor:
    if x.dtype == torch.bfloat16:
        from . import ops_bf16
        return ops_bf16.PermuteRows16.apply(x, idx, scatter)
    return _PermuteRows.apply(x, idx, scatter)


class _Axpby(torch.autograd.Function):
    @staticmethod
    def forward(ctx, x, y, a: float, b: float):
        _capi.require_device(x, y)
        ctx.a, ctx.b = a, b
        return _axpby_raw(a, x, b, y)

    @staticmethod
    def backward(ctx, g):
        g = g.contiguous()
        return _axpby_raw(ctx.a, g), _axpby_raw(ctx.b, g), None, None


def axpby(a: float, x: Tensor, b: float, y: Tensor) -> Tensor:
    return _Axpby.apply(x, y, a, b)


@dataclasses.dataclass
class Seg:

    t: Tensor
    idx: Optional[Tensor] = None
    relu: bool = False
    reduce: object = None


@dataclasses.dataclass
class _MlpSpec:
    n_seg: int
    n_layers: int
    has_bias: bool
    idx: list
    relu: list
    reduce: list
    epilogue: int
    ca: float
    cb: float
    out_idx: Optional[Tensor]
    out_rows: int
    n_rows: int
    grad_on: bool

    @staticmethod
    def of(segs: Sequence[Seg], weights, biases, *, n_rows: int, epilogue: int = _capi.EPI_NONE, ca: float = 0.0,
           cb: float = 1.0, out_idx: Optional[Tensor] = None, out_rows: Optional[int] = None) -> "_MlpSpec":
        return _MlpSpec(len(segs), len(weights), any(b is not None for b in biases),
                        [s.idx for s in segs], [s.relu for s in segs], [s.reduce for s in segs],
                        epilogue, float(ca), float(cb), out_idx, int(n_rows if out_rows is None else out_rows),
                        int(n_rows), torch.is_grad_enabled())


def _fill_mlp(weights: Sequence[Tensor], biases: Sequence[Optional[Tensor]]):
    n_layers = len(weights)
    hidden = weights[0].shape[0]
    in_dim = weights[0].shape[1]
    out_dim = weights[-1].shape[0]
    if n_layers not in (2, 3):
        raise NotImplementedError(
            f"fused MLP kernels cover L=2 and L=3 (the reference's uses); got L={n_layers}")
    for i, w in enumerate(weights):
        exp = (hidden if i < n_layers - 1 else out_dim, in_dim if i == 0 else hidden)
        if tuple(w.shape) != exp:
            raise ValueError(f"layer {i} weight has shape {tuple(w.shape)}, expected {exp}")
    if in_dim > _capi.MAX_IN_BF16 or hidden > _capi.MAX_HIDDEN_BF16 or out_dim > _capi.MAX_OUT_BF16:
        raise NotImplementedError(
            f"fused MLP kernel limits: in<={_capi.MAX_IN_BF16}, hidden<={_capi.MAX_HIDDEN_BF16}, "
            f"out<={_capi.MAX_OUT_BF16}; got in={in_dim}, hidden={hidden}, out={out_dim}")
    return _capi.make_mlp([_p(w) for w in weights], [_p(b) for b in biases], in_dim, hidden,
                          out_dim)


_GRAD_SINK = os.environ.get("GNNTRK_GRAD_SINK", "1") != "0"
_SINKS_ARMED = 0


@contextlib.contextmanager
def grad_sinks_armed():
    global _SINKS_ARMED
    _SINKS_ARMED += 1
    try:
        yield
    finally:
        _SINKS_ARMED -= 1


def _param_grad_sinks(weights, biases, need_w, need_b):
    if not _GRAD_SINK or _SINKS_ARMED <= 0:
        return None
    gW, gb = [], []
    for plist, need, out in ((weights, need_w, gW), (biases, need_b, gb)):
        for p_, nd in zip(plist, need):
            if p_ is None:
                out.append(None)
                continue
            g = getattr(p_, "grad", None)
            if (not nd or not getattr(p_, "_gnntrk_grad_sink", False) or g is None or g.dtype != torch.float32
                    or g.shape != p_.shape or g.device != p_.device or not g.is_contiguous()
                    or getattr(p_, "_backward_hooks", None) or getattr(p_, "_post_accumulate_grad_hooks", None)):
                return None
            out.append(g)
    return gW, gb


def _unpack(spec: _MlpSpec, tensors, as_rows):
    ns, nl = spec.n_seg, spec.n_layers
    segs = [as_rows(t) for t in tensors[:ns]]
    weights = [w.contiguous() for w in tensors[ns:ns + nl]]
    biases = [None if b is None else b.contiguous() for b in tensors[ns + nl:ns + 2 * nl]]
    res = tensors[ns + 2 * nl] if len(tensors) > ns + 2 * nl else None
    _capi.require_device(*segs, *weights)
    mlp = _fill_mlp(weights, biases)
    if sum(s.shape[1] for s in segs) != mlp.in_dim:
        raise AssertionError(
            f"Expected feature dimension {mlp.in_dim}, got {sum(s.shape[1] for s in segs)}")
    return segs, weights, biases, res, mlp


def _save(ctx, spec: _MlpSpec, segs, weights, biases, *extras) -> None:
    ctx.spec = spec
    ctx.save_for_backward(*extras, *segs, *weights, *[b for b in biases if b is not None])
    ctx.bias_mask = [b is not None for b in biases]


def _restore(ctx, n_extra: int = 0):
    ns, nl = ctx.spec.n_seg, ctx.spec.n_layers
    saved = ctx.saved_tensors
    segs, weights = list(saved[n_extra:n_extra + ns]), list(saved[n_extra + ns:n_extra + ns + nl])
    rest = iter(saved[n_extra + ns + nl:])
    biases = [next(rest) if m else None for m in ctx.bias_mask]
    return saved[:n_extra], segs, weights, biases, _fill_mlp(weights, biases)


def _fill_args(a, mlp, segs, idx, relu, seg_of, n_rows: int, epilogue: int, ca: float, cb: float):
    a.mlp = mlp
    a.n_seg, a.epilogue, a.n_rows = len(segs), epilogue, n_rows
    a.ca, a.cb = ca, cb
    for j, s in enumerate(segs):
        a.seg[j] = seg_of(s, idx[j], relu[j])
    return a


def _seg32(t: Tensor, idx, relu: bool):
    return _capi.Seg(_p(t), _p(idx), t.shape[1], _row_stride(t), int(relu), 0)


def _param_grad_plan(weights, biases, need):
    if not any(need):
        return False, None
    nl = len(weights)
    return True, _param_grad_sinks(weights, biases, need[:nl], [need[nl + i] or biases[i] is None for i in range(nl)])


def _param_grad_fill(a, weights, biases, want_dw: bool, sinks):
    nl = len(weights)
    if not want_dw:
        return [None] * nl, [None] * nl
    if sinks is not None:
        gW, gb = sinks
    else:
        gW = [torch.empty_like(w) for w in weights]
        gb = [None if b is None else torch.empty_like(b) for b in biases]
    for i in range(nl):
        a.gW[i] = _p(gW[i])
        a.gb[i] = _p(gb[i])
    a.accumulate_params = 1 if sinks is not None else 0
    return gW, gb


def _param_grad_outs(need, gW, gb, sinks) -> list:
    if sinks is not None:
        return [None] * len(need)
    return [g if n else None for g, n in zip([*gW, *gb], need)]


def _require_reduce(reduce):
    if reduce is None:
        raise RuntimeError("gathered segment requires a `reduce` rule for backward")
    return reduce


def _fold_rows(rows: Tensor, idx: Tensor, reduce, n_src: int) -> Tensor:
    if reduce == "perm":
        return _permute_raw(rows, idx, scatter=True)
    by, gi = _require_reduce(reduce)
    return _segment_sum_raw(rows, *_fold_of(by, gi), n_src)


def _sum_terms(gterms) -> Tensor:
    total = None
    for g, idx in gterms:
        rows = g if idx is None else _permute_raw(g, idx, scatter=False)
        total = rows if total is None else total + rows
    return total.contiguous()


_Fp32Kernels = collections.namedtuple("_Fp32Kernels", "forward backward n_extra tall_identity")
_DEBUG_FLAGS = int(os.environ.get("GNNTRK_DEBUG_FLAGS", "0"))


def _reg_forward(lib, a, spec, segs, out, keep):
    M = spec.n_rows
    nbytes = M * (sum(4 * s.shape[1] + (4 if spec.idx[j] is not None else 0)
                      for j, s in enumerate(segs)) + 4 * a.mlp.out_dim
                  + (4 if spec.out_idx is not None else 0)
                  + (4 * a.mlp.out_dim if spec.epilogue == _capi.EPI_RESIDUAL else 0))
    with _timed(out, kernel_key(lib, a, False), _mlp_flops_per_row(a.mlp) * M, nbytes, M):
        _capi.check(lib.gnntrk_mlp_forward(C.byref(a), _stream(out)), lib)
    return ()


def _reg_backward(lib, a, spec, segs, need_seg, want_dw, g0, extras):
    ws = _ws(lib.gnntrk_mlp_backward_workspace_bytes(C.byref(a.mlp)), g0) if want_dw else None
    a.debug_flags = _DEBUG_FLAGS
    M = spec.n_rows
    nbytes = M * (sum(4 * s.shape[1] + (4 if spec.idx[j] is not None else 0)
                      + (4 * s.shape[1] if need_seg[j] else 0)
                      for j, s in enumerate(segs)) + 4 * a.mlp.out_dim
                  + (4 if spec.out_idx is not None else 0))
    with _timed(g0, kernel_key(lib, a, True), 3 * _mlp_flops_per_row(a.mlp) * M, nbytes, M):
        _capi.check(lib.gnntrk_mlp_backward(C.byref(a), _p(ws), 0 if ws is None else ws.numel(), _stream(g0)), lib)


def _wide_forward(lib, a, spec, segs, out, keep):
    M = spec.n_rows
    acts = None
    if keep and M > 0:
        hp = int(lib.gnntrk_mlp_wide_hidden_pad(a.mlp.hidden))
        acts = torch.empty(spec.n_layers - 1, M, hp, dtype=torch.float32, device=out.device)
    ws = _ws(lib.gnntrk_mlp_wide_forward_workspace_bytes(C.byref(a.mlp)), out)
    _capi.check(lib.gnntrk_mlp_forward_wide(C.byref(a), _p(acts), _p(ws), ws.numel(), _stream(out)), lib)
    return acts, out if spec.epilogue == _capi.EPI_RELU else None


def _wide_backward(lib, a, spec, segs, need_seg, want_dw, g0, extras):
    acts, out = extras
    ws = _ws(lib.gnntrk_mlp_wide_backward_workspace_bytes(C.byref(a.mlp), spec.n_rows), g0)
    _capi.check(lib.gnntrk_mlp_backward_wide(C.byref(a), _p(acts), _p(out), 0 if out is None else _row_stride(out),
                                             _p(ws), ws.numel(), _stream(g0)), lib)


_REG = _Fp32Kernels(_reg_forward, _reg_backward, 0, True)
_WIDE = _Fp32Kernels(_wide_forward, _wide_backward, 2, False)


def _fp32_forward(ctx, kernels: _Fp32Kernels, spec: _MlpSpec, tensors) -> Tensor:
    segs, weights, biases, res, mlp = _unpack(spec, tensors, _as_rows)
    lib = _capi.load()
    a = _fill_args(_capi.MlpFwdArgs(), mlp, segs, spec.idx, spec.relu, _seg32, spec.n_rows, spec.epilogue,
                   spec.ca, spec.cb)
    if spec.epilogue == _capi.EPI_RESIDUAL:
        res = _as_rows(res)
        a.res, a.res_stride = _p(res), _row_stride(res)
    out = torch.empty(spec.out_rows, mlp.out_dim, dtype=torch.float32, device=segs[0].device)
    a.out, a.out_stride, a.out_idx = _p(out), _row_stride(out), _p(spec.out_idx)
    extras = kernels.forward(lib, a, spec, segs, out, spec.grad_on and any(ctx.needs_input_grad))
    _save(ctx, spec, segs, weights, biases, *extras)
    return out


def _fp32_backward(ctx, kernels: _Fp32Kernels, gterms, need):
    spec: _MlpSpec = ctx.spec
    ns, nl = spec.n_seg, spec.n_layers
    extras, segs, weights, biases, mlp = _restore(ctx, kernels.n_extra)
    lib = _capi.load()
    gterms = [(_as_rows(g.contiguous()), idx) for g, idx in gterms]
    g0 = gterms[0][0]
    a = _fill_args(_capi.MlpBwdArgs(), mlp, segs, spec.idx, spec.relu, _seg32, spec.n_rows, spec.epilogue,
                   spec.ca, spec.cb)
    a.n_gout = len(gterms)
    for t, (g, idx) in enumerate(gterms):
        a.gout[t] = _capi.GTerm(_p(g), _p(idx), _row_stride(g), 0)
    M = spec.n_rows
    need_seg = [bool(n) for n in need[1:1 + ns]]
    seg_grads: list[Optional[Tensor]] = [None] * ns
    row_tmp: list[Optional[Tensor]] = [None] * ns
    for j, s in enumerate(segs):
        if not need_seg[j]:
            continue
        if spec.idx[j] is None:
            if s.shape[0] != M and not kernels.tall_identity:
                raise RuntimeError("identity segments must have n_rows rows")
            gj = seg_grads[j] = torch.empty(s.shape[0], s.shape[1], dtype=torch.float32, device=g0.device)
            if s.shape[0] != M:
                gj.zero_()
        else:
            _require_reduce(spec.reduce[j])
            gj = row_tmp[j] = torch.empty(M, s.shape[1], dtype=torch.float32, device=g0.device)
        a.gseg[j] = _capi.GSeg(_p(gj), None, _row_stride(gj), 0)
    need_p = need[1 + ns:1 + ns + 2 * nl]
    want_dw, sinks = _param_grad_plan(weights, biases, need_p)
    gW, gb = _param_grad_fill(a, weights, biases, want_dw, sinks)
    kernels.backward(lib, a, spec, segs, need_seg, want_dw, g0, extras)
    for j, s in enumerate(segs):
        if row_tmp[j] is None:
            continue
        if spec.reduce[j] == "perm" and s.shape[0] != M:
            raise RuntimeError("'perm' segments must cover all source rows")
        seg_grads[j] = _fold_rows(row_tmp[j], spec.idx[j], spec.reduce[j], s.shape[0])
    g_res = None
    if spec.epilogue == _capi.EPI_RESIDUAL and need[1 + ns + 2 * nl]:
        g_res = _axpby_raw(spec.ca, _sum_terms(gterms))
    return (None, *seg_grads, *_param_grad_outs(need_p, gW, gb, sinks), g_res)


class _FusedMLP(torch.autograd.Function):
    @staticmethod
    def forward(ctx, spec: _MlpSpec, *tensors):
        return _fp32_forward(ctx, _REG, spec, tensors)

    @staticmethod
    def backward(ctx, g_out):
        return _fp32_backward(ctx, _REG, [(g_out, ctx.spec.out_idx)], ctx.needs_input_grad)


class _FusedMLPWide(torch.autograd.Function):

    @staticmethod
    def forward(ctx, spec: _MlpSpec, *tensors):
        return _fp32_forward(ctx, _WIDE, spec, tensors)

    @staticmethod
    def backward(ctx, g_out):
        return _fp32_backward(ctx, _WIDE, [(g_out, None)], ctx.needs_input_grad)


class _FusedINEdgeWide(torch.autograd.Function):

    @staticmethod
    def forward(ctx, spec: _MlpSpec, gi: GraphIndex, *tensors):
        e_tilde = _fp32_forward(ctx, _WIDE, spec, tensors)
        ctx.gi = gi
        ctx.set_materialize_grads(False)
        return e_tilde, _segment_sum_raw(e_tilde, gi.rowptr_t, None, gi.n_nodes)

    @staticmethod
    def backward(ctx, g_et, g_aggr):
        gterms = []
        if g_et is not None:
            gterms.append((g_et, None))
        if g_aggr is not None:
            gterms.append((g_aggr, ctx.gi.tgt))
        need = ctx.needs_input_grad
        if not gterms:
            return (None,) * len(need)
        outs = _fp32_backward(ctx, _WIDE, gterms, (need[0],) + tuple(need[2:]) + (False,))
        return (None, None, *outs[1:-1])


def in_edge_wide(segs, weights, biases, gi: GraphIndex, n_rows: int):
    spec = _MlpSpec.of(segs, weights, biases, n_rows=n_rows)
    return _FusedINEdgeWide.apply(spec, gi, *[s.t for s in segs], *weights, *biases)


def fused_mlp(segs: Sequence[Seg], weights: Sequence[Tensor],
              biases: Sequence[Optional[Tensor]], *, n_rows: Optional[int] = None,
              epilogue: int = _capi.EPI_NONE, ca: float = 0.0, cb: float = 1.0,
              res: Optional[Tensor] = None, out_idx: Optional[Tensor] = None,
              out_rows: Optional[int] = None) -> Tensor:
    if not 1 <= len(segs) <= _capi.MAX_SEGS:
        raise ValueError(f"1..{_capi.MAX_SEGS} segments supported, got {len(segs)}")
    if n_rows is None:
        s0 = segs[0]
        n_rows = int(s0.idx.shape[0]) if s0.idx is not None else int(s0.t.shape[0])
    for s in segs:
        if s.t.dim() == 1:
            raise ValueError("fused_mlp segments must be 2-D [rows, dim]")
    bf16 = segs[0].t.dtype == torch.bfloat16
    if _fused_supported(segs, weights, biases, bf16, epilogue):
        node = _FusedMLP
        if bf16:
            from . import ops_bf16
            node = ops_bf16.FusedMLP16
    elif not bf16 and out_idx is None and _wide_kernel_supported(segs, weights, epilogue):
        node, out_rows = _FusedMLPWide, None
    else:
        return _wide_mlp(segs, weights, biases, n_rows=int(n_rows), epilogue=epilogue, ca=float(ca), cb=float(cb),
                         res=res, out_idx=out_idx, out_rows=int(out_rows if out_rows is not None else n_rows))
    spec = _MlpSpec.of(segs, weights, biases, n_rows=n_rows, epilogue=epilogue, ca=ca, cb=cb, out_idx=out_idx,
                       out_rows=out_rows)
    return node.apply(spec, *[s.t for s in segs], *weights, *biases, res)


_FUSED_HEAD_LOSS = os.environ.get("GNNTRK_FUSED_HEAD_LOSS", "1") != "0"
_HEAD_DEFERRAL = None


class _HeadDeferral:

    def __init__(self, scale: float):
        self.scale, self.loss = float(scale), None


@contextlib.contextmanager
def head_loss_deferral(scale: float = 1.0, enabled: bool = True):
    global _HEAD_DEFERRAL
    old = _HEAD_DEFERRAL
    _HEAD_DEFERRAL = _HeadDeferral(scale) if (enabled and _FUSED_HEAD_LOSS) else None
    try:
        yield _HEAD_DEFERRAL
    finally:
        _HEAD_DEFERRAL = old


def head_deferral_active() -> bool:
    return _HEAD_DEFERRAL is not None and _HEAD_DEFERRAL.loss is None and torch.is_grad_enabled()


def deferred_head(segs: Sequence[Seg], weights: Sequence[Tensor], biases, gi: "GraphIndex", y, *, n_rows: int,
                  ca: float, cb: float, head):
    from .edge_order import PendingEdgeWeights

    if (not head_deferral_active() or n_rows < 2 or not isinstance(y, Tensor) or carried_label(gi, y) is None
            or not 1 <= len(segs) <= _capi.MAX_SEGS or any(s.t.dim() != 2 or s.t.dtype != torch.bfloat16 for s in segs)
            or int(weights[-1].shape[0]) != 1 or len(weights) != 3
            or not _fused_supported(segs, weights, biases, True, _capi.EPI_SIGMOID)
            or not any(t is not None and t.requires_grad for t in [s.t for s in segs] + list(weights) + list(biases))):
        return None
    spec = _MlpSpec.of(segs, weights, biases, n_rows=n_rows, epilogue=_capi.EPI_SIGMOID, ca=ca, cb=cb)
    return PendingEdgeWeights(n_rows, segs[0].t.device, gi, head,
                              (spec, [s.t for s in segs], list(weights), list(biases)))


def _fused_head_loss(w, y: Tensor, edge_index: Optional[Tensor], pt_thld: float) -> Optional[Tensor]:
    from .edge_order import PendingEdgeWeights

    d = _HEAD_DEFERRAL
    if (not isinstance(w, PendingEdgeWeights) or not w.pending or d is None or d.loss is not None
            or pt_thld > 0.0 or not torch.is_grad_enabled() or not _edge_index_is_index_source(w.graph_index, edge_index)):
        return None
    gi = w.graph_index
    lab = carried_label(gi, y)
    if lab is None:
        return None
    from . import ops_bf16

    w_buf = torch.empty(gi.n_edges, dtype=torch.float32, device=lab.device)
    loss = torch.empty(1, dtype=torch.float32, device=lab.device)
    spec, seg_t, weights, biases = w.take_fused(w_buf)
    bce = ops_bf16.HeadBce(lab, w_buf, loss, d.scale, done=w.filled)
    d.loss = ops_bf16.HeadBCE16.apply(spec, bce, *seg_t, *weights, *biases)
    return d.loss


_BF16_MAX_CHUNKS = 32


def _fused_supported(segs: Sequence[Seg], weights: Sequence[Tensor], biases, bf16: bool, epilogue=None) -> bool:
    L = len(weights)
    if L not in (2, 3):
        return False
    hidden, out_dim = int(weights[0].shape[0]), int(weights[-1].shape[0])
    in_dim = sum(int(s.t.shape[1]) if s.t.dim() == 2 else 1 for s in segs)
    chunks = sum((int(s.t.shape[1]) + 3) // 4 for s in segs if s.t.dim() == 2)
    if out_dim > (_capi.MAX_OUT_BF16 if bf16 else _capi.MAX_OUT):
        return False
    if bf16:
        has_bias = any(b is not None for b in biases)
        spare = any(int(s.t.shape[1]) % 4 for s in segs if s.t.dim() == 2)
        n_ch = chunks + (1 if has_bias and not spare else 0)
        hid_bias = any(b is not None for b in list(biases)[1:])
        rows = hidden + (1 if hid_bias and not (hidden == 64 or (hidden == 128 and n_ch <= 8)) else 0)
        if out_dim > 16 or n_ch > 16:
            return (n_ch <= _BF16_MAX_CHUNKS and 33 <= rows <= 48
                    and epilogue in (None, _capi.EPI_NONE, _capi.EPI_RESIDUAL))
        return n_ch <= 16 and rows <= (128 if n_ch <= 8 else 96)
    return in_dim <= _capi.MAX_IN and hidden <= _capi.MAX_HIDDEN and chunks <= 16


_WIDE_KERNEL = os.environ.get("GNNTRK_WIDE_KERNEL", "1") != "0"


def _wide_kernel_supported(segs: Sequence[Seg], weights: Sequence[Tensor], epilogue) -> bool:
    if not _WIDE_KERNEL or len(weights) not in (2, 3):
        return False
    if any(s.t.dtype != torch.float32 for s in segs) or any(w.dtype != torch.float32 for w in weights):
        return False
    hidden, out_dim = int(weights[0].shape[0]), int(weights[-1].shape[0])
    in_dim = sum(int(s.t.shape[1]) for s in segs)
    return (in_dim <= _capi.WIDE_MAX_IN and hidden <= _capi.WIDE_MAX_HIDDEN and out_dim <= _capi.WIDE_MAX_OUT
            and epilogue in (None, _capi.EPI_NONE, _capi.EPI_RELU, _capi.EPI_RESIDUAL))


class _GatherRows(torch.autograd.Function):

    @staticmethod
    def forward(ctx, t, idx, reduce):
        ctx.idx, ctx.reduce, ctx.n, ctx.dt = idx, reduce, int(t.shape[0]), t.dtype
        return t.index_select(0, idx.long())

    @staticmethod
    def backward(ctx, g):
        out = _fold_rows(g.to(torch.float32).contiguous(), ctx.idx, ctx.reduce, ctx.n)
        return out.to(ctx.dt), None, None


_WIDE_WARNED: set = set()


def _wide_mlp(segs: Sequence[Seg], weights, biases, *, n_rows: int, epilogue: int, ca: float, cb: float,
              res: Optional[Tensor], out_idx: Optional[Tensor], out_rows: int) -> Tensor:
    import torch.nn.functional as F

    bf16 = segs[0].t.dtype == torch.bfloat16
    shape = (sum(int(s.t.shape[1]) for s in segs), *[int(w.shape[0]) for w in weights])
    if shape not in _WIDE_WARNED:
        _WIDE_WARNED.add(shape)
        import logging
        logging.getLogger("gnn_tracking_amd").info(
            "MLP %s is outside the fused kernels' shapes; running it as library GEMMs", "->".join(map(str, shape)))
    _capi.require_device(*[s.t for s in segs])
    cols = []
    for s_ in segs:
        t = s_.t
        if s_.relu:
            t = torch.relu(t)
        if s_.idx is not None:
            t = _GatherRows.apply(t, s_.idx, s_.reduce)
        cols.append(t)
    x = cols[0] if len(cols) == 1 else torch.cat(cols, dim=1)
    if x.shape[0] != n_rows:
        raise ValueError(f"segments have {x.shape[0]} rows, expected {n_rows}")
    dt = torch.bfloat16 if bf16 else torch.float32
    L = len(weights)
    for i, (w, b) in enumerate(zip(weights, biases)):
        x = F.linear(x.to(dt), w.to(dt), None if b is None else b.to(dt))
        if i < L - 1:
            x = torch.relu(x)
    if epilogue == _capi.EPI_RELU:
        x = torch.relu(x)
    elif epilogue == _capi.EPI_RESIDUAL:
        x = ca * res.to(x.dtype) + cb * x
    elif epilogue == _capi.EPI_SIGMOID:
        x = ca + cb * torch.sigmoid(x.float())
    if out_idx is not None:
        if out_rows != n_rows:
            raise ValueError("out_idx must be a permutation of the rows")
        x = permute_rows(x.contiguous(), out_idx, scatter=True)
    if bf16 and x.dtype == torch.bfloat16:
        d, pad = int(x.shape[1]), (-int(x.shape[1])) % 4
        x = F.pad(x, (0, pad))[:, :d] if pad else x.contiguous()
    return x


_KNN_FLAGS = int(os.environ.get("GNNTRK_KNN_FLAGS", "0"))


def _radius_admits_nothing(max_radius: Optional[float]) -> bool:
    return max_radius is not None and not (max_radius > 0)


def _knn_search(lib, x: Tensor, k: int, r: float, seg_ptr: Optional[Tensor], nbr: Tensor, cnt: Tensor, st) -> None:
    n, dim = int(x.shape[0]), int(x.shape[1])
    nb = int(lib.gnntrk_knn_workspace_bytes(n, dim, k))
    ws = torch.empty(nb, dtype=torch.uint8, device=x.device) if nb else None
    n_seg = int(seg_ptr.numel()) - 1 if seg_ptr is not None else 0
    _capi.check(lib.gnntrk_knn_search_ws(_p(x), n, dim, _row_stride(x), k, r,
                                         _p(seg_ptr) if seg_ptr is not None else None, n_seg, _p(nbr), _p(cnt),
                                         _p(ws) if ws is not None else None, nb, _KNN_FLAGS, st), lib)


def knn_graph(x: Tensor, k: int, max_radius: Optional[float] = None, seg_ptr: Optional[Tensor] = None) -> Tensor:
    _capi.require_device(x)
    lib = _capi.load()
    if x.dim() != 2:
        raise ValueError("knn_graph: x must be [N, D]")
    x = _as_rows(x.detach())
    n, dim = int(x.shape[0]), int(x.shape[1])
    dev = x.device
    if n <= 1 or _radius_admits_nothing(max_radius):
        return torch.empty(2, 0, dtype=torch.int64, device=dev)
    kk = min(int(k), n - 1)
    nbr = torch.empty(n * kk, dtype=torch.int32, device=dev)
    cnt = torch.empty(n, dtype=torch.int32, device=dev)
    st = _stream(x)
    r = float(max_radius) if max_radius is not None else -1.0
    sp = seg_ptr.to(device=dev, dtype=torch.int64).contiguous() if seg_ptr is not None else None
    _knn_search(lib, x, kk, r, sp, nbr, cnt, st)
    off = torch.empty(n + 1, dtype=torch.int64, device=dev)
    _capi.check(lib.gnntrk_knn_emit(_p(nbr), _p(cnt), n, kk, _p(off), None, 0, st), lib)
    m = int(off[n].item())
    ei = torch.empty(2, m, dtype=torch.int64, device=dev)
    _capi.check(lib.gnntrk_knn_emit(_p(nbr), _p(cnt), n, kk, _p(off), _p(ei), m, st), lib)
    return ei


def knn_kth_neighbor(x: Tensor, k: int, max_radius: Optional[float] = None, seg_ptr: Optional[Tensor] = None) -> Tensor:
    _capi.require_device(x)
    lib = _capi.load()
    x = _as_rows(x.detach().to(torch.float32))
    n, dim = int(x.shape[0]), int(x.shape[1])
    if n - 1 < k or _radius_admits_nothing(max_radius):
        return torch.full((n,), -1, dtype=torch.int32, device=x.device)
    nbr = torch.empty(n * k, dtype=torch.int32, device=x.device)
    cnt = torch.empty(n, dtype=torch.int32, device=x.device)
    r = float(max_radius) if max_radius is not None else -1.0
    sp = seg_ptr.to(device=x.device, dtype=torch.int64).contiguous() if seg_ptr is not None else None
    _knn_search(lib, x, int(k), r, sp, nbr, cnt, _stream(x))
    last = nbr.view(n, k)[:, k - 1]
    return torch.where(cnt >= k, last, torch.full_like(last, -1)).contiguous()


def max_radius_count(x: Tensor, radius: float) -> Tensor:
    _capi.require_device(x)
    lib = _capi.load()
    x = _as_rows(x.detach().to(torch.float32))
    n, dim = int(x.shape[0]), int(x.shape[1])
    if n < 2:
        return torch.zeros((), dtype=torch.int32, device=x.device)
    cnt = torch.empty(n, dtype=torch.int32, device=x.device)
    off = torch.empty(n + 1, dtype=torch.int64, device=x.device)
    nb = int(lib.gnntrk_radius_points_workspace_bytes(n, dim))
    ws = torch.empty(nb, dtype=torch.uint8, device=x.device) if nb else None
    _capi.check(lib.gnntrk_radius_count_ws(_p(x), n, dim, _row_stride(x), float(radius), _p(cnt), _p(off),
                                           _p(ws) if ws is not None else None, nb, 0, _stream(x)), lib)
    return cnt.max() - 1


def knn_scan(x: Tensor, ks: Sequence[int], max_radius: Optional[float] = None) -> dict:
    _capi.require_device(x)
    lib = _capi.load()
    if x.dim() != 2:
        raise ValueError("knn_scan: x must be [N, D]")
    ks = [int(k) for k in ks]
    if not ks or min(ks) < 1:
        raise ValueError("knn_scan: ks must be positive")
    x = _as_rows(x.detach())
    n, dim = int(x.shape[0]), int(x.shape[1])
    dev = x.device
    if n <= 1 or _radius_admits_nothing(max_radius):
        return {k: torch.empty(2, 0, dtype=torch.int64, device=dev) for k in ks}
    kmax = min(max(ks), n - 1)
    nbr = torch.empty(n * kmax, dtype=torch.int32, device=dev)
    cnt = torch.empty(n, dtype=torch.int32, device=dev)
    st = _stream(x)
    r = float(max_radius) if max_radius is not None else -1.0
    _knn_search(lib, x, kmax, r, None, nbr, cnt, st)
    offs = {}
    for k in ks:
        off = torch.empty(n + 1, dtype=torch.int64, device=dev)
        _capi.check(lib.gnntrk_knn_emit_prefix(_p(nbr), _p(cnt), n, kmax, min(k, kmax), _p(off), None, 0, st), lib)
        offs[k] = off
    totals = torch.stack([offs[k][n] for k in ks]).tolist()
    out = {}
    for k, m in zip(ks, totals):
        ei = torch.empty(2, int(m), dtype=torch.int64, device=dev)
        _capi.check(lib.gnntrk_knn_emit_prefix(_p(nbr), _p(cnt), n, kmax, min(k, kmax), _p(offs[k]), _p(ei),
                                               int(m), st), lib)
        out[k] = ei
    return out


def edge_labels(particle_id: Tensor, edge_index: Tensor) -> Tensor:
    _capi.require_device(particle_id, edge_index)
    lib = _capi.load()
    pid = particle_id.to(torch.int64).contiguous()
    ei = edge_index.contiguous()
    m = int(ei.shape[1])
    y = torch.empty(m, dtype=torch.int64, device=ei.device)
    _capi.check(lib.gnntrk_edge_labels(_p(pid), _p(ei), m, _p(y), _stream(ei)), lib)
    return y


class _EdgeFeatures(torch.autograd.Function):
    @staticmethod
    def forward(ctx, x, edge_index):
        lib = _capi.load()
        x2 = _as_rows(x.detach())
        ei = edge_index.contiguous()
        m, f = int(ei.shape[1]), int(x2.shape[1])
        out = torch.empty(m, 2 * f, dtype=torch.float32, device=x2.device)
        _capi.check(lib.gnntrk_edge_features(_p(x2), f, _row_stride(x2), _p(ei), m, _p(out),
                                             _stream(x2)), lib)
        ctx.ei, ctx.n, ctx.f = edge_index, int(x2.shape[0]), f
        return out

    @staticmethod
    def backward(ctx, g):
        f, n = ctx.f, ctx.n
        gi = graph_index(ctx.ei, n)
        g0 = _permute_raw((g[:, :f] + g[:, f:]).contiguous(), gi.perm, scatter=False)
        g1 = _permute_raw((g[:, f:] - g[:, :f]).contiguous(), gi.perm, scatter=False)
        gx = _segment_sum_raw(g1, gi.rowptr_t, None, n)
        _segment_sum_raw(g0, gi.rowptr_s, gi.spos, n, out=gx, accumulate=True)
        return gx, None


def edge_features(x: Tensor, edge_index: Tensor) -> Tensor:
    _capi.require_device(x, edge_index)
    if x.dtype != torch.float32:
        x = x.float()
    return _EdgeFeatures.apply(x, edge_index)


class _BCE(torch.autograd.Function):
    @staticmethod
    def forward(ctx, w, y, src_nodes, pt, pt_thld: float):
        _capi.require_device(w, y)
        lib = _capi.load()
        w = w.contiguous().view(-1)
        y = y.contiguous().view(-1)
        n = w.numel()
        loss = torch.empty(1, dtype=torch.float32, device=w.device)
        ws = _ws(lib.gnntrk_bce_workspace_bytes(n), w)
        _capi.check(lib.gnntrk_bce_forward(_p(w), _p(y), _p(src_nodes), _p(pt), pt_thld, n,
                                           _p(loss), _p(ws), ws.numel(), _stream(w)), lib)
        ctx.save_for_backward(w, y)
        ctx.aux = (src_nodes, pt, pt_thld)
        return loss.view(())

    @staticmethod
    def backward(ctx, g):
        lib = _capi.load()
        w, y = ctx.saved_tensors
        src_nodes, pt, thld = ctx.aux
        g = g.contiguous().view(1).to(torch.float32)
        gw = torch.empty_like(w)
        _capi.check(lib.gnntrk_bce_backward(_p(w), _p(y), _p(src_nodes), _p(pt), thld, w.numel(),
                                            _p(g), _p(gw), _stream(w)), lib)
        return gw, None, None, None, None


class _BCECsr(torch.autograd.Function):

    @staticmethod
    def forward(ctx, w, label_csr, src_csr, pt, pt_thld: float):
        _capi.require_device(w, label_csr)
        lib = _capi.load()
        w = w.contiguous().view(-1)
        n = w.numel()
        loss = torch.empty(1, dtype=torch.float32, device=w.device)
        gw = torch.empty_like(w) if ctx.needs_input_grad[0] else None
        ws = _ws(lib.gnntrk_bce_workspace_bytes(n), w)
        _capi.check(lib.gnntrk_bce_csr(_p(w), _p(label_csr), _p(src_csr), _p(pt), pt_thld, n, _p(loss), _p(gw),
                                       _p(ws), ws.numel(), _stream(w)), lib)
        ctx.save_for_backward(*([gw] if gw is not None else []))
        return loss.view(())

    @staticmethod
    def backward(ctx, g):
        (gw,) = ctx.saved_tensors
        return gw * g.to(torch.float32), None, None, None, None


class _Focal(torch.autograd.Function):
    @staticmethod
    def forward(ctx, w, y, src_nodes, pt, pt_thld: float, alpha: float, gamma: float, pos_weight: float,
                haughty: bool):
        _capi.require_device(w, y)
        lib = _capi.load()
        w = w.contiguous().view(-1)
        y = y.contiguous().view(-1)
        n = w.numel()
        loss = torch.empty(1, dtype=torch.float32, device=w.device)
        ws = _ws(lib.gnntrk_bce_workspace_bytes(n), w)
        _capi.check(lib.gnntrk_focal_forward(_p(w), _p(y), _p(src_nodes), _p(pt), pt_thld, alpha, gamma, pos_weight,
                                             int(haughty), n, _p(loss), _p(ws), ws.numel(), _stream(w)), lib)
        ctx.save_for_backward(w, y)
        ctx.aux = (src_nodes, pt, pt_thld, alpha, gamma, pos_weight, int(haughty))
        return loss.view(())

    @staticmethod
    def backward(ctx, g):
        lib = _capi.load()
        w, y = ctx.saved_tensors
        src_nodes, pt, thld, alpha, gamma, pos_weight, haughty = ctx.aux
        g = g.contiguous().view(1).to(torch.float32)
        gw = torch.empty_like(w)
        _capi.check(lib.gnntrk_focal_backward(_p(w), _p(y), _p(src_nodes), _p(pt), thld, alpha, gamma, pos_weight,
                                              haughty, w.numel(), _p(g), _p(gw), _stream(w)), lib)
        return gw, None, None, None, None, None, None, None, None


def edge_targets_csr(y: Tensor, gi: GraphIndex, pt: Optional[Tensor] = None, pt_thld: float = 0.0) -> Tensor:
    key = (id(y), y._version, None if pt is None else id(pt), float(pt_thld))
    hit = getattr(gi, "_targets", None)
    if hit is not None and hit[0] == key and hit[1]() is y:
        return hit[2]
    _capi.require_device(y)
    lib = _capi.load()
    u8 = y.dtype in (torch.bool, torch.uint8)
    yf = (y.detach().view(torch.uint8) if u8 else y.detach().to(torch.float32)).contiguous().view(-1)
    if yf.numel() != gi.n_edges:
        raise ValueError(f"labels have {yf.numel()} entries, the graph has {gi.n_edges} edges")
    ptf = None
    if pt_thld > 0.0:
        assert pt is not None
        ptf = gi.node_values(pt.detach().to(torch.float32)).contiguous()
    out = torch.empty(gi.n_edges, dtype=torch.float32, device=yf.device)
    _capi.check(lib.gnntrk_edge_targets_csr(_p(yf), int(u8), _p(gi.perm), _p(gi.src), _p(ptf), float(pt_thld),
                                            gi.n_edges, _p(out), _stream(yf)), lib)
    gi._targets = (key, weakref.ref(y), out)
    return out


def _csr_fast_path(w, edge_index):
    from .edge_order import EdgeOrdered

    if not isinstance(w, EdgeOrdered):
        return None
    gi = w.graph_index
    if not _edge_index_is_index_source(gi, edge_index):
        return None
    return w.csr.reshape(-1), gi


def _edge_index_is_index_source(gi, edge_index) -> bool:
    if edge_index is not None:
        if int(edge_index.shape[1]) != gi.n_edges:
            return False
        src = getattr(gi, "_built_from", None)
        if src is not None and not (src[0]() is edge_index and src[1] == edge_index._version):
            return False
    return True


def focal_loss(w: Tensor, y: Tensor, edge_index: Optional[Tensor] = None, pt: Optional[Tensor] = None,
               pt_thld: float = 0.0, *, alpha: float = 0.25, gamma: float = 2.0, pos_weight: float = 1.0,
               haughty: bool = False) -> Tensor:
    if w.numel() == 0:
        return w.sum() * float("nan")
    if w.dtype != torch.float32:
        raise TypeError("focal_loss: w must be fp32")
    assert gamma >= 0.0
    assert 0 <= alpha <= 1
    fast = None if haughty else _csr_fast_path(w, edge_index)
    if fast is not None:
        w_csr, gi = fast
        t = edge_targets_csr(y, gi, pt, float(pt_thld))
        return _Focal.apply(w_csr, t, None, None, 0.0, float(alpha), float(gamma), float(pos_weight), False)
    y = y.to(torch.float32)
    src_nodes = None
    if pt_thld > 0.0:
        assert edge_index is not None and pt is not None
        src_nodes = edge_index[0].contiguous()
        pt = pt.to(torch.float32).contiguous()
    else:
        pt = None
    return _Focal.apply(w, y, src_nodes, pt, float(pt_thld), float(alpha), float(gamma), float(pos_weight),
                        bool(haughty))


def bce_loss(w: Tensor, y: Tensor, edge_index: Optional[Tensor] = None,
             pt: Optional[Tensor] = None, pt_thld: float = 0.0) -> Tensor:
    if w.numel() == 0:
        return w.sum() * float("nan")
    if w.dtype != torch.float32:
        raise TypeError("bce_loss: w must be fp32")
    fused = _fused_head_loss(w, y, edge_index, float(pt_thld))
    if fused is not None:
        return fused
    fast = _csr_fast_path(w, edge_index)
    if fast is not None:
        w_csr, gi = fast
        lab = carried_label(gi, y)
        if lab is not None:
            ptf = None
            if pt_thld > 0.0:
                assert pt is not None
                ptf = pt.detach().to(torch.float32).contiguous()
                if ptf.device != w_csr.device or ptf.numel() < gi.n_nodes:
                    raise ValueError(f"bce_loss: pt must hold one value per node ({gi.n_nodes}) on {w_csr.device}, "
                                     f"got {ptf.numel()} on {ptf.device}")
                ptf = gi.node_values(ptf).contiguous()
            return _BCECsr.apply(w_csr, lab, gi.src if pt_thld > 0.0 else None, ptf, float(pt_thld))
        return _BCE.apply(w_csr, edge_targets_csr(y, gi, pt, float(pt_thld)), None, None, 0.0)
    y = y.to(torch.float32)
    src_nodes = None
    if pt_thld > 0.0:
        assert edge_index is not None and pt is not None
        src_nodes = edge_index[0].contiguous()
        pt = pt.to(torch.float32).contiguous()
    else:
        pt = None
    return _BCE.apply(w, y, src_nodes, pt, float(pt_thld))
```

Before: 3.024 billion.

## Piggyback source-key histogram and partitioning onto first CSR sort pass

Adds a 'ride' mode in which the first (target-keyed) count pass also builds a global histogram of source keys. The first sort's output stage then scatters source-keyed records directly into pre-scanned source partitions, staged through LDS windows. This lets the second (source-keyed) sort skip its own zeroing, count and split work when no bucket overflows; an over flag gates those kernels as a fallback. It costs extra atomics, shared memory and workspace in the first pass, and it is only enabled when nodes are ordered or renumbered.

```diff
diff --git a/gnn_tracking_amd/csrc/graph_index.hip b/gnn_tracking_amd/csrc/graph_index.hip
--- a/gnn_tracking_amd/csrc/graph_index.hip
+++ b/gnn_tracking_amd/csrc/graph_index.hip
@@ -60,6 +60,19 @@
         } else {
 #pragma unroll
             for (int q = 0; q < 4; ++q) k[q] = e + q < e1 ? key(e + q, bad) : 0u;
+        }
+    }
+    __device__ __forceinline__ void pays4(int64_t e, int64_t e1, uint32_t p[4]) const {
+        if (vec && e + 4 <= e1) {
+            const longlong2 a = *reinterpret_cast<const longlong2 *>(src + e);
+            const longlong2 b = *reinterpret_cast<const longlong2 *>(src + e + 2);
+            p[0] = checked(a.x, nullptr);
+            p[1] = checked(a.y, nullptr);
+            p[2] = checked(b.x, nullptr);
+            p[3] = checked(b.y, nullptr);
+        } else {
+#pragma unroll
+            for (int q = 0; q < 4; ++q) p[q] = e + q < e1 ? checked(src[e + q], nullptr) : 0u;
         }
     }
     struct Raw {
@@ -163,7 +176,7 @@
 __device__ __forceinline__ void gi_remap4(const int64_t *__restrict__ src, const int64_t *__restrict__ tgt, int64_t e,
                                           int64_t e1, int64_t N, const int32_t *__restrict__ rank, int vec,
                                           int32_t *__restrict__ src32, int32_t *__restrict__ tgt32,
-                                          int *__restrict__ bad, uint32_t kt[4]) {
+                                          int *__restrict__ bad, uint32_t kt[4], uint32_t ks[4]) {
     if (vec && e + 4 <= e1) {
         typedef int i4_hw __attribute__((ext_vector_type(4)));
         auto ld2 = [](const int64_t *p, long long &a, long long &b) {
@@ -186,16 +199,20 @@
         __builtin_nontemporal_store(ot, reinterpret_cast<i4_hw *>(tgt32 + e));
         __builtin_nontemporal_store(os, reinterpret_cast<i4_hw *>(src32 + e));
 #pragma unroll
-        for (int q = 0; q < 4; ++q) kt[q] = (uint32_t)ot[q];
+        for (int q = 0; q < 4; ++q) {
+            kt[q] = (uint32_t)ot[q];
+            ks[q] = (uint32_t)os[q];
+        }
     } else {
 #pragma unroll
         for (int q = 0; q < 4; ++q) {
-            kt[q] = 0u;
+            kt[q] = ks[q] = 0u;
             if (e + q < e1) {
                 const int t = rank[gi_clamped<false>(tgt[e + q], N, bad)], u = rank[gi_clamped<false>(src[e + q], N, bad)];
                 tgt32[e + q] = t;
                 src32[e + q] = u;
                 kt[q] = (uint32_t)t;
+                ks[q] = (uint32_t)u;
             }
         }
     }
@@ -285,58 +302,107 @@
     __syncthreads();
     if (tid == 0) range[c] = int2{*s_lo, *s_hi};
 }
-template <class K>
+__device__ __forceinline__ void gi_tot4(const uint32_t s4[4], int64_t e, int64_t e1, int w0s, uint32_t *s_tot,
+                                        uint32_t *__restrict__ tot) {
+#pragma unroll
+    for (int q = 0; q < 4; ++q) {
+        if (e + q >= e1) break;
+        const uint32_t b = s4[q] >> kSH, d = b - (uint32_t)w0s;
+        if (d < (uint32_t)kWin)
+            atomicAdd(&s_tot[d], 1u);
+        else
+            atomicAdd(&tot[b], 1u);
+    }
+}
+template <int TPB>
+__device__ __forceinline__ void gi_tot_flush(const uint32_t *s_tot, int w0s, uint32_t *__restrict__ tot) {
+    __syncthreads();
+    for (int d = threadIdx.x; d < kWin; d += TPB) {
+        const uint32_t v = s_tot[d];
+        if (v) atomicAdd(&tot[w0s + d], v);
+    }
+}
+template <class K, bool RIDE>
 __global__ __launch_bounds__(kCountTpb) void gi_count_kernel(K keys, int64_t E, int chunk, int n_chunks, int NB,
                                                              uint32_t *__restrict__ tbl, int2 *__restrict__ range,
-                                                             int *__restrict__ bad) {
+                                                             int *__restrict__ bad, uint32_t *__restrict__ tot,
+                                                             const int *__restrict__ gate) {
     __shared__ uint32_t s_cnt[kWin];
+    __shared__ uint32_t s_tot[RIDE ? kWin : 1];
     __shared__ int s_lo, s_hi;
+    if (gate && *gate == 0) return;
     const int tid = threadIdx.x, c = blockIdx.x;
     const int64_t e0 = (int64_t)c * chunk, e1 = e0 + chunk < E ? e0 + chunk : E;
-    for (int d = tid; d < kWin; d += kCountTpb) s_cnt[d] = 0;
+    for (int d = tid; d < kWin; d += kCountTpb) {
+        s_cnt[d] = 0;
+        if (RIDE) s_tot[d] = 0;
+    }
     if (tid == 0) {
         s_lo = kWin;
         s_hi = -1;
     }
     __syncthreads();
     const int w0 = gi_window_start(keys.key(e0, nullptr));
+    int w0s = 0;
+    if constexpr (RIDE) {
+        uint32_t f4[4];
+        keys.pays4(e0, e0 + 1, f4);
+        w0s = gi_window_start(f4[0]);
+    }
     for (int64_t e = e0 + 4 * tid; e < e1; e += 4 * kCountTpb) {
         uint32_t k4[4];
         keys.keys4(e, e1, k4, bad);
         gi_count4(k4, e, e1, w0, s_cnt, tbl, n_chunks, c);
+        if constexpr (RIDE) {
+            uint32_t s4[4];
+            keys.pays4(e, e1, s4);
+            gi_tot4(s4, e, e1, w0s, s_tot, tot);
+        }
     }
     gi_count_flush<kCountTpb>(s_cnt, &s_lo, &s_hi, w0, n_chunks, c, tbl, range);
+    if (RIDE) gi_tot_flush<kCountTpb>(s_tot, w0s, tot);
     (void)NB;
 }
 constexpr int kRemapTpb = 1024;
+template <bool RIDE>
 __global__ __launch_bounds__(kRemapTpb, 8) void gi_remap_count_kernel(
     const int64_t *__restrict__ src, const int64_t *__restrict__ tgt, int64_t E, int64_t N,
     const int32_t *__restrict__ rank, int vec, int32_t *__restrict__ src32, int32_t *__restrict__ tgt32, int chunk,
-    int n_chunks, uint32_t *__restrict__ tbl, int2 *__restrict__ range, int *__restrict__ bad) {
+    int n_chunks, uint32_t *__restrict__ tbl, int2 *__restrict__ range, int *__restrict__ bad,
+    uint32_t *__restrict__ tot) {
     __shared__ uint32_t s_cnt[kWin];
-    __shared__ int s_lo, s_hi, s_w0;
+    __shared__ uint32_t s_tot[RIDE ? kWin : 1];
+    __shared__ int s_lo, s_hi, s_w0, s_w0s;
     const int tid = threadIdx.x, c = gi_chunk_of_block();
     if (c >= n_chunks) return;
     const int64_t e0 = (int64_t)c * chunk, e1 = e0 + chunk < E ? e0 + chunk : E;
-    for (int d = tid; d < kWin; d += kRemapTpb) s_cnt[d] = 0;
+    for (int d = tid; d < kWin; d += kRemapTpb) {
+        s_cnt[d] = 0;
+        if (RIDE) s_tot[d] = 0;
+    }
     if (tid == 0) {
         s_lo = kWin;
         s_hi = -1;
         s_w0 = gi_window_start((uint32_t)rank[gi_clamped<true>(tgt[e0], N, nullptr)]);
-    }
-    __syncthreads();
-    const int w0 = s_w0;
+        s_w0s = RIDE ? gi_window_start((uint32_t)rank[gi_clamped<true>(src[e0], N, nullptr)]) : 0;
+    }
+    __syncthreads();
+    const int w0 = s_w0, w0s = s_w0s;
     for (int64_t e = e0 + 4 * tid; e < e1; e += 4 * kRemapTpb) {
-        uint32_t k4[4];
-        gi_remap4(src, tgt, e, e1, N, rank, vec, src32, tgt32, bad, k4);
+        uint32_t k4[4], s4[4];
+        gi_remap4(src, tgt, e, e1, N, rank, vec, src32, tgt32, bad, k4, s4);
         gi_count4(k4, e, e1, w0, s_cnt, tbl, n_chunks, c);
+        if (RIDE) gi_tot4(s4, e, e1, w0s, s_tot, tot);
     }
     gi_count_flush<kRemapTpb>(s_cnt, &s_lo, &s_hi, w0, n_chunks, c, tbl, range);
+    if (RIDE) gi_tot_flush<kRemapTpb>(s_tot, w0s, tot);
 }
 
 __global__ __launch_bounds__(kScanTpb) void gi_scan_sums_kernel(const uint32_t *__restrict__ v, int64_t n,
-                                                                uint32_t *__restrict__ sums) {
+                                                                uint32_t *__restrict__ sums,
+                                                                const int *__restrict__ gate) {
     __shared__ uint32_t s[kScanTpb];
+    if (gate && *gate == 0) return;
     const int tid = threadIdx.x;
     const int64_t i0 = (int64_t)blockIdx.x * kScanTile + (int64_t)tid * kScanItems;
     uint32_t t = 0;
@@ -360,9 +426,11 @@
 
 __global__ __launch_bounds__(kScanTpb) void gi_scan_apply_kernel(uint32_t *__restrict__ v, int64_t n,
                                                                  const uint32_t *__restrict__ sums, int n_chunks,
-                                                                 uint32_t *__restrict__ base) {
+                                                                 uint32_t *__restrict__ base,
+                                                                 const int *__restrict__ gate) {
     __shared__ uint32_t s[kScanTpb];
     __shared__ uint32_t s_before[kScanTpb / 64];
+    if (gate && *gate == 0) return;
     const int tid = threadIdx.x;
     const int64_t i0 = (int64_t)blockIdx.x * kScanTile + (int64_t)tid * kScanItems;
     uint32_t before = 0;
@@ -423,6 +491,7 @@
     }
 }
 
+template <int TPB = kSplitTpb>
 __device__ __forceinline__ uint32_t gi_block_exscan(uint32_t v, uint32_t *s_wsum, uint32_t *total) {
     const int tid = threadIdx.x, lane = tid & 63, wv = tid >> 6;
     uint32_t inc = v;
@@ -435,7 +504,7 @@
     __syncthreads();
     uint32_t pre = 0, tot = 0;
 #pragma unroll
-    for (int w = 0; w < kSplitTpb / 64; ++w) {
+    for (int w = 0; w < TPB / 64; ++w) {
         const uint32_t t = s_wsum[w];
         pre += w < wv ? t : 0u;
         tot += t;
@@ -443,6 +512,40 @@
     __syncthreads();
     *total = tot;
     return pre + inc - v;
+}
+__global__ __launch_bounds__(kSplitTpb) void gi_ride_scan_kernel(uint32_t *__restrict__ tot, int NB,
+                                                                 uint32_t *__restrict__ base_s, int *__restrict__ over) {
+    __shared__ uint32_t s_wsum[kSplitTpb / 64];
+    const int tid = threadIdx.x;
+    uint32_t before = 0, mx = 0;
+    for (int t0 = 0; t0 < NB; t0 += 4 * kSplitTpb) {
+        const int i0 = t0 + 4 * tid;
+        uint32_t v[4], sum = 0;
+#pragma unroll
+        for (int q = 0; q < 4; ++q) {
+            v[q] = i0 + q < NB ? tot[i0 + q] : 0u;
+            sum += v[q];
+            mx = v[q] > mx ? v[q] : mx;
+        }
+        uint32_t total;
+        uint32_t run = before + gi_block_exscan(sum, s_wsum, &total);
+#pragma unroll
+        for (int q = 0; q < 4; ++q) {
+            if (i0 + q < NB) {
+                base_s[i0 + q] = run;
+                tot[i0 + q] = run;
+            }
+            run += v[q];
+        }
+        before += total;
+    }
+    if (tid == 0) base_s[NB] = before;
+    if (mx > (uint32_t)kCap) *over = 1;
+}
+__global__ __launch_bounds__(kTpb) void gi_zero_kernel(uint4 *__restrict__ v, int64_t n16, const int *__restrict__ gate) {
+    if (gate && *gate == 0) return;
+    for (int64_t i = (int64_t)blockIdx.x * kTpb + threadIdx.x; i < n16; i += (int64_t)gridDim.x * kTpb)
+        v[i] = uint4{0u, 0u, 0u, 0u};
 }
 
 template <bool ROWS>
@@ -462,13 +565,14 @@
                                                              uint32_t *__restrict__ tbl,
                                                              const int2 *__restrict__ range,
                                                              typename GiRec<ROWS>::type *__restrict__ part,
-                                                             int *__restrict__ bad) {
+                                                             int *__restrict__ bad, const int *__restrict__ gate) {
     typedef typename GiRec<ROWS>::type Rec;
     __shared__ uint32_t s_off[kWin];
     __shared__ uint32_t s_cnt[kWin];
     __shared__ Rec s_stage[kSplitTile];
     __shared__ uint16_t s_slot[kSplitTile];
     __shared__ uint32_t s_wsum[kSplitTpb / 64];
+    if (gate && *gate == 0) return;
     const int tid = threadIdx.x, c = blockIdx.x;
     const int64_t e0 = (int64_t)c * chunk, e1 = e0 + chunk < E ? e0 + chunk : E;
     const int w0 = gi_window_start(keys.key(e0, nullptr));
@@ -555,19 +659,30 @@
     }
 }
 
+constexpr int kRideWin = 1024;
 template <bool ROWS>
 struct OutCsr {
     static constexpr uint32_t kValMask = 0x7fffffffu;
     static constexpr bool kRows = ROWS;
+    static constexpr bool kCanEmit = true;
     int32_t *perm, *tgt, *src, *rowptr;
     uint32_t pmask;
     uint8_t *label_csr;
     uint16_t *rows_csr;
     int rows_out_stride;
-    __device__ __forceinline__ void ranked(uint32_t k, uint32_t val, uint32_t hi) const {
+    uint32_t *cur_s;
+    uint2 *part_s;
+    const int *over;
+    __device__ __forceinline__ bool emits() const { return cur_s != nullptr && *over == 0; }
+    __device__ __forceinline__ uint32_t source(uint32_t hi) const { return hi & pmask; }
+    __device__ __forceinline__ void emit_one(uint32_t k, uint32_t s) const {
+        part_s[atomicAdd(&cur_s[s >> kSH], 1u)] = uint2{k, s & (uint32_t)(kBins - 1)};
+    }
+    __device__ __forceinline__ void ranked(uint32_t k, uint32_t val, uint32_t hi, bool emit) const {
         perm[k] = (int32_t)(val & kValMask);
         src[k] = (int32_t)(hi & pmask);
         if (label_csr) label_csr[k] = (uint8_t)(val >> 31);
+        if (emit) emit_one(k, hi & pmask);
     }
     __device__ __forceinline__ void row(uint32_t k, uint2 r) const {
         if (ROWS) *reinterpret_cast<uint2 *>(rows_csr + (size_t)k * rows_out_stride) = r;
@@ -578,8 +693,12 @@
 struct OutSrc {
     static constexpr uint32_t kValMask = 0xffffffffu;
     static constexpr bool kRows = false;
+    static constexpr bool kCanEmit = false;
     int32_t *spos, *spos_inv, *rowptr;
-    __device__ __forceinline__ void ranked(uint32_t k, uint32_t val, uint32_t) const {
+    __device__ __forceinline__ bool emits() const { return false; }
+    __device__ __forceinline__ uint32_t source(uint32_t) const { return 0u; }
+    __device__ __forceinline__ void emit_one(uint32_t, uint32_t) const {}
+    __device__ __forceinline__ void ranked(uint32_t k, uint32_t val, uint32_t, bool) const {
         spos[k] = (int32_t)val;
         if (spos_inv) spos_inv[val] = (int32_t)k;
     }
@@ -593,11 +712,18 @@
 template <class O>
 constexpr uint32_t kGiCapG = O::kRows ? (uint32_t)kCap * 2 / 3 : (uint32_t)kCap;
 
+template <bool ON>
+struct GiRideLds {
+    uint32_t cnt[ON ? kRideWin : 1];
+    uint32_t off[ON ? kRideWin : 1];
+    uint32_t wsum[kSortTpb / 64];
+    int lo;
+};
 template <class O>
 __device__ __forceinline__ void gi_sort_fits(uint2 (&rec)[kSortR], const uint2 (&rrow)[O::kRows ? kSortR : 1],
                                              uint32_t (&ord)[kSortR], uint32_t base, uint32_t M, uint32_t node0,
                                              int pbits, const uint32_t *s_hist, const uint32_t *s_start, uint2 *s_rec,
-                                             uint16_t *s_fin, const O &out) {
+                                             uint16_t *s_fin, GiRideLds<O::kCanEmit> *rl, bool emit, const O &out) {
     constexpr uint32_t VM = O::kValMask;
     const int tid = threadIdx.x;
 #pragma unroll
@@ -628,9 +754,38 @@
     for (int q = 0; q < kSortR; ++q)
         if (tid + q * kSortTpb < M) s_rec[dst[q]] = rec[q];
     __syncthreads();
-    for (uint32_t j = tid; j < M; j += kSortTpb) {
-        const uint2 r = s_rec[j];
-        out.ranked(base + j, r.x, r.y);
+    uint32_t em[O::kCanEmit ? kSortR : 1], n_in = 0;
+    if (!(O::kCanEmit && emit))
+        for (uint32_t j = tid; j < M; j += kSortTpb) {
+            const uint2 r = s_rec[j];
+            out.ranked(base + j, r.x, r.y, false);
+        }
+    if constexpr (O::kCanEmit) {
+        if (emit) {
+            static_assert(kRideWin == 2 * kSortTpb && kRideWin <= 1024 && kCap <= 8192, "two slots per thread; em[] packing");
+            const uint32_t lo = (uint32_t)rl->lo;
+#pragma unroll
+            for (int q = 0; q < kSortR; ++q) {
+                const uint32_t j = tid + q * kSortTpb;
+                em[q] = 0u;
+                if (j < M) {
+                    const uint2 r = s_rec[j];
+                    out.ranked(base + j, r.x, r.y, false);
+                    const uint32_t s = out.source(r.y), d = (s >> kSH) - lo;
+                    if (d < (uint32_t)kRideWin)
+                        em[q] = 0x80000000u | (d << 21) | (atomicAdd(&rl->cnt[d], 1u) << 8) | (s & (uint32_t)(kBins - 1));
+                    else
+                        out.emit_one(base + j, s);
+                }
+            }
+            __syncthreads();
+            const uint32_t c0 = rl->cnt[2 * tid], c1 = rl->cnt[2 * tid + 1];
+            const uint32_t l0 = gi_block_exscan<kSortTpb>(c0 + c1, rl->wsum, &n_in), l1 = l0 + c0;
+            rl->cnt[2 * tid] = l0;
+            rl->cnt[2 * tid + 1] = l1;
+            if (c0) rl->off[2 * tid] = atomicAdd(&out.cur_s[lo + 2 * tid], c0) - l0;
+            if (c1) rl->off[2 * tid + 1] = atomicAdd(&out.cur_s[lo + 2 * tid + 1], c1) - l1;
+        }
     }
     if (O::kRows) {
         __syncthreads();
@@ -639,6 +794,23 @@
             if (tid + q * kSortTpb < M) s_rec[s_fin[ord[q]]] = rrow[O::kRows ? q : 0];
         __syncthreads();
         for (uint32_t j = tid; j < M; j += kSortTpb) out.row(base + j, s_rec[j]);
+    }
+    if constexpr (O::kCanEmit) {
+        if (emit) {
+            __syncthreads();
+#pragma unroll
+            for (int q = 0; q < kSortR; ++q)
+                if (em[q] >> 31) {
+                    const uint32_t d = (em[q] >> 21) & (uint32_t)(kRideWin - 1);
+                    s_rec[rl->cnt[d] + ((em[q] >> 8) & 0x1fffu)] =
+                        uint2{base + (uint32_t)tid + (uint32_t)q * kSortTpb, (d << 8) | (em[q] & 0xffu)};
+                }
+            __syncthreads();
+            for (uint32_t j = tid; j < n_in; j += kSortTpb) {
+                const uint2 r = s_rec[j];
+                out.part_s[rl->off[r.y >> 8] + j] = uint2{r.x, r.y & 0xffu};
+            }
+        }
     }
 }
 
@@ -649,6 +821,7 @@
     constexpr uint32_t VM = O::kValMask, kRS = kGiRS<O>;
     const int tid = threadIdx.x;
     uint32_t *s_pos32 = reinterpret_cast<uint32_t *>(s_rec + kGiCapG<O>);
+    const bool emit = O::kCanEmit && out.emits();
     const uint32_t st0 = s_start[g0], n_g = (g1 < kBins ? s_start[g1] : M) - st0;
     __syncthreads();
     if (tid < kBins) s_cur[tid] = 0;
@@ -668,7 +841,7 @@
         const uint32_t low = r.y >> pbits, st = s_start[low] - st0, n = s_hist[low];
         uint32_t cnt = 0;
         for (uint32_t t = 0; t < n; ++t) cnt += (s_rec[st + t].x & VM) < (r.x & VM) ? 1u : 0u;
-        out.ranked(base + st0 + st + cnt, r.x, r.y);
+        out.ranked(base + st0 + st + cnt, r.x, r.y, emit);
         if (O::kRows) out.row(base + st0 + st + cnt, part[(size_t)s_pos32[j] * kRS + (kRS - 1)]);
         out.slot(base + st0 + j, node0 + low);
     }
@@ -706,6 +879,7 @@
                                             int chunk, int g0, const uint32_t *h_all, const uint32_t *h_hub,
                                             const O &out) {
     constexpr uint32_t VM = O::kValMask, kRS = kGiRS<O>;
+    const bool emit = O::kCanEmit && out.emits();
     for (uint32_t i = threadIdx.x; i < M; i += kSortTpb) {
         const uint2 r = part[(size_t)i * kRS];
         if ((int)(r.y >> pbits) != g0) continue;
@@ -716,7 +890,7 @@
             const uint2 q = part[(size_t)t * kRS];
             cnt += ((int)(q.y >> pbits) == g0 && (q.x & VM) < (r.x & VM)) ? 1u : 0u;
         }
-        out.ranked(pos0 + cnt, r.x, r.y);
+        out.ranked(pos0 + cnt, r.x, r.y, emit);
         if (O::kRows) out.row(pos0 + cnt, part[(size_t)i * kRS + (kRS - 1)]);
     }
 }
@@ -727,6 +901,7 @@
                                                const uint32_t *h_hub, uint32_t *bm, uint32_t *pw, const O &out) {
     constexpr uint32_t VM = O::kValMask, kRS = kGiRS<O>, kSpanW = kHubSpanW, kSpan = kHubSpan;
     const int tid = threadIdx.x;
+    const bool emit = O::kCanEmit && out.emits();
     for (int ck = 0; ck < kMaxChunks; ++ck) {
         const uint32_t r0 = h_all[ck], r1 = ck + 1 < kMaxChunks ? h_all[ck + 1] : M;
         const uint32_t hub_here = (ck + 1 < kMaxChunks ? h_hub[ck + 1] : n) - h_hub[ck];
@@ -769,7 +944,7 @@
                 if ((int)(q.y >> pbits) == g0 && d < kSpan) {
                     const uint32_t w = d >> 5;
                     const uint32_t below = (uint32_t)__popc(bm[w] & ((1u << (d & 31u)) - 1u));
-                    out.ranked(pos0 + before + pw[w] + below, q.x, q.y);
+                    out.ranked(pos0 + before + pw[w] + below, q.x, q.y, emit);
                     if (O::kRows) out.row(pos0 + before + pw[w] + below, part[(size_t)t * kRS + (kRS - 1)]);
                 }
             }
@@ -781,18 +956,31 @@
 template <class O>
 __global__ __launch_bounds__(kSortTpb) void gi_bucket_sort_kernel(const typename GiRec<O::kRows>::type *__restrict__ part_,
                                                                   const uint32_t *__restrict__ base_arr, int NB,
-                                                                  int64_t N, int64_t E, int pbits, int chunk, O out) {
+                                                                  int64_t N, int64_t E, int pbits, int chunk, O out,
+                                                                  const typename GiRec<O::kRows>::type *__restrict__ part_rode,
+                                                                  const uint32_t *__restrict__ base_rode,
+                                                                  const int *__restrict__ gate) {
     constexpr uint32_t kRS = kGiRS<O>;
-    const uint2 *__restrict__ part = reinterpret_cast<const uint2 *>(part_);
     __shared__ uint32_t s_hist[kBins], s_start[kBins], s_wsum[kBins / 64], s_cur[kBins];
     __shared__ uint2 s_rec[kCap];
     __shared__ uint16_t s_fin[O::kRows ? kCap : 1];
+    __shared__ GiRideLds<O::kCanEmit> s_ride;
+    if (gate && *gate == 0) {
+        part_ = part_rode;
+        base_arr = base_rode;
+    }
+    const uint2 *__restrict__ part = reinterpret_cast<const uint2 *>(part_);
     const int tid = threadIdx.x, b = blockIdx.x, lane = tid & 63, wv = tid >> 6;
     const uint32_t base = base_arr[b], M = base_arr[b + 1] - base;
     part += (size_t)base * kRS;
     const uint32_t node0 = (uint32_t)b << kSH;
     const bool fits = M <= (uint32_t)kCap;
+    const bool emit = O::kCanEmit && out.emits();
     if (tid < kBins) s_hist[tid] = 0;
+    if (O::kCanEmit && emit) {
+        for (int d = tid; d < kRideWin; d += kSortTpb) s_ride.cnt[d] = 0;
+        if (tid == 0) s_ride.lo = 0x7fffffff;
+    }
     __syncthreads();
     uint2 rec[kSortR], rrow[O::kRows ? kSortR : 1];
     uint32_t ord[kSortR];
@@ -811,6 +999,20 @@
 #pragma unroll
         for (int q = 0; q < kSortR; ++q)
             if (tid + q * kSortTpb < M) ord[q] = atomicAdd(&s_hist[rec[q].y >> pbits], 1u);
+        if (O::kCanEmit && emit) {
+            uint32_t mn = 0x7fffffffu;
+#pragma unroll
+            for (int q = 0; q < kSortR; ++q)
+                if (tid + q * kSortTpb < M) {
+                    const uint32_t sb = out.source(rec[q].y) >> kSH;
+                    mn = sb < mn ? sb : mn;
+                }
+            for (int o = 32; o > 0; o >>= 1) {
+                const uint32_t t = (uint32_t)__shfl_xor((int)mn, o);
+                mn = t < mn ? t : mn;
+            }
+            if (lane == 0) atomicMin(&s_ride.lo, (int)mn);
+        }
     } else {
         for (uint32_t i = tid; i < M; i += kSortTpb) atomicAdd(&s_hist[part[(size_t)i * kRS].y >> pbits], 1u);
     }
@@ -838,7 +1040,7 @@
     if (b == NB - 1 && tid == 0) out.node_start(N, (uint32_t)E);
     __syncthreads();
     if (fits) {
-        gi_sort_fits(rec, rrow, ord, base, M, node0, pbits, s_hist, s_start, s_rec, s_fin, out);
+        gi_sort_fits(rec, rrow, ord, base, M, node0, pbits, s_hist, s_start, s_rec, s_fin, &s_ride, emit, out);
     } else {
         int g0 = 0;
         while (g0 < kBins) {
@@ -875,6 +1077,7 @@
     int64_t T;
     int n_tiles;
     size_t off_range, off_base, off_tbl, off_sums, off_part, bytes;
+    size_t off_tot, off_base_s;
 };
 
 static int bits_for(int64_t n) {
@@ -883,7 +1086,7 @@
     return b;
 }
 
-static OwnPlan own_plan(int64_t N, int64_t E, bool rows) {
+static OwnPlan own_plan(int64_t N, int64_t E, bool rows, bool ride = false) {
     OwnPlan p{};
     p.ok = false;
     if (N < 1 || E < 1) return p;
@@ -901,6 +1104,12 @@
     p.dense = E / p.NB > kCap * 9 / 10;
     p.n_tiles = (int)ceil_div(p.T + 1, kScanTile);
     size_t o = kHeader;
+    if (ride) {
+        p.off_tot = o;
+        o += align_up((size_t)(p.NB + 1) * 4, 256);
+        p.off_base_s = o;
+        o += align_up((size_t)(p.NB + 1) * 4, 256);
+    }
     p.off_tbl = o;
     o += align_up((size_t)(p.T + 1) * 4, 256);
     p.off_range = o;
@@ -924,28 +1133,32 @@
                      "counting sort(memset)");
 }
 
-template <class K>
-static void own_count(const OwnPlan &p, K keys, int64_t E, char *ws, int *bad, hipStream_t stream) {
-    hipLaunchKernelGGL((gi_count_kernel<K>), dim3(p.n_chunks), dim3(kCountTpb), 0, stream, keys, E, p.chunk,
-                       p.n_chunks, p.NB, own_tbl(p, ws), own_range(p, ws), bad);
+template <class K, bool RIDE = false>
+static void own_count(const OwnPlan &p, K keys, int64_t E, char *ws, int *bad, hipStream_t stream,
+                      const int *gate = nullptr) {
+    hipLaunchKernelGGL((gi_count_kernel<K, RIDE>), dim3(p.n_chunks), dim3(kCountTpb), 0, stream, keys, E, p.chunk,
+                       p.n_chunks, p.NB, own_tbl(p, ws), own_range(p, ws), bad,
+                       RIDE ? reinterpret_cast<uint32_t *>(ws + p.off_tot) : nullptr, gate);
 }
 
 template <class K, class O>
 static void own_sort(const OwnPlan &p, K keys, O out, int pbits, int64_t N, int64_t E, char *ws, int *bad,
-                     hipStream_t stream) {
+                     hipStream_t stream, const int *gate = nullptr,
+                     const typename GiRec<O::kRows>::type *part_rode = nullptr) {
     typedef typename GiRec<O::kRows>::type Rec;
     int2 *range = own_range(p, ws);
     uint32_t *tbl = own_tbl(p, ws);
     uint32_t *base = reinterpret_cast<uint32_t *>(ws + p.off_base);
     uint32_t *sums = reinterpret_cast<uint32_t *>(ws + p.off_sums);
     Rec *part = reinterpret_cast<Rec *>(ws + p.off_part);
-    hipLaunchKernelGGL(gi_scan_sums_kernel, dim3(p.n_tiles), dim3(kScanTpb), 0, stream, tbl, p.T + 1, sums);
+    hipLaunchKernelGGL(gi_scan_sums_kernel, dim3(p.n_tiles), dim3(kScanTpb), 0, stream, tbl, p.T + 1, sums, gate);
     hipLaunchKernelGGL(gi_scan_apply_kernel, dim3(p.n_tiles), dim3(kScanTpb), 0, stream, tbl, p.T + 1, sums,
-                       p.n_chunks, base);
+                       p.n_chunks, base, gate);
     hipLaunchKernelGGL((gi_split_kernel<K, O::kRows>), dim3(p.n_chunks), dim3(kSplitTpb), 0, stream, keys, E, p.chunk,
-                       p.n_chunks, pbits, tbl, range, part, bad);
+                       p.n_chunks, pbits, tbl, range, part, bad, gate);
     hipLaunchKernelGGL((gi_bucket_sort_kernel<O>), dim3(p.NB), dim3(kSortTpb), 0, stream, part, base, p.NB, N, E,
-                       pbits, p.chunk, out);
+                       pbits, p.chunk, out, part_rode,
+                       gate ? reinterpret_cast<const uint32_t *>(ws + p.off_base_s) : nullptr, gate);
 }
 
 __device__ __forceinline__ uint32_t gi_checked(int64_t v, int64_t N, const int32_t *rank, int *bad) {
@@ -1012,8 +1225,8 @@
 static size_t remap_arr_bytes(int64_t E) { return align_up((size_t)(E > 0 ? E : 1) * sizeof(int32_t), 256); }
 static size_t graph_index_ws_bytes(int64_t N, int64_t E, int carry) {
     const size_t lib = library_ws_bytes(E);
-    const OwnPlan p = own_plan(N, E, (carry & 1) != 0);
-    const size_t own = p.ok ? align_up(p.bytes, 256) + ((carry & 2) ? 2 * remap_arr_bytes(E) : 0) : 0;
+    const OwnPlan p = own_plan(N, E, (carry & 1) != 0, (carry & 4) != 0);
+    const size_t own = p.ok ? align_up(p.bytes, 256) + ((carry & 6) ? 2 * remap_arr_bytes(E) : 0) : 0;
     return own > lib ? own : lib;
 }
 
@@ -1076,13 +1289,14 @@
         return fail(GNNTRK_EINVAL,
                     "graph_index_build: carried rows must be 16-byte aligned fp32 [E, 4] with a row stride that is a "
                     "multiple of 4 floats; the bf16 output 8-byte aligned with a stride that is a multiple of 4");
-    if (!ws || ws_bytes < graph_index_ws_bytes(N, E, (rows ? 1 : 0) | (rank ? 2 : 0)))
+    const bool ride = (flags & 16) != 0;
+    if (!ws || ws_bytes < graph_index_ws_bytes(N, E, (rows ? 1 : 0) | (rank ? 2 : 0) | (ride ? 4 : 0)))
         return fail(GNNTRK_EINVAL, "graph_index_build: workspace too small");
 
     char *p = reinterpret_cast<char *>(ws);
     int *bad = reinterpret_cast<int *>(p);
     int rc = GNNTRK_OK;
-    const OwnPlan plan = own_plan(N, E, rows != nullptr);
+    const OwnPlan plan = own_plan(N, E, rows != nullptr, ride);
     const bool own = E > 0 && plan.ok && !(flags & 1) && (!plan.dense || (flags & 2));
     if (!own) {
         rc = check_hip(hipMemsetAsync(bad, 0, kHeader, stream), "graph_index_build(memset)");
@@ -1094,37 +1308,55 @@
                             (!label || ((uintptr_t)label & 3) == 0);
             const KeysCoo k1{edge_index, edge_index + E, N, label, rows, rows ? cy->rows_stride : 0, vec, nullptr};
             const uint32_t pmask = (uint32_t)(((uint64_t)1 << plan.bitsN) - 1);
+            uint32_t *tot_s = ride ? reinterpret_cast<uint32_t *>(p + plan.off_tot) : nullptr;
+            uint2 *part_s = ride ? reinterpret_cast<uint2 *>(p + align_up(plan.bytes, 256)) : nullptr;
+            int *over = ride ? bad + 1 : nullptr;
             const OutCsr<true> o1r{o->perm, o->tgt, o->src, o->rowptr_t, pmask, label ? cy->label_csr : nullptr,
-                                   rows ? cy->rows_csr_bf16 : nullptr, rows ? cy->out_stride : 0};
+                                   rows ? cy->rows_csr_bf16 : nullptr, rows ? cy->out_stride : 0, tot_s, part_s, over};
             const OutCsr<false> o1{o->perm, o->tgt, o->src, o->rowptr_t, pmask, label ? cy->label_csr : nullptr,
-                                   nullptr, 0};
+                                   nullptr, 0, tot_s, part_s, over};
             auto first_sort = [&](auto keys) {
+                if (ride)
+                    hipLaunchKernelGGL(gi_ride_scan_kernel, dim3(1), dim3(kSplitTpb), 0, stream, tot_s, plan.NB,
+                                       reinterpret_cast<uint32_t *>(p + plan.off_base_s), over);
                 if (rows)
                     own_sort(plan, keys, o1r, plan.bitsN, N, E, p, bad, stream);
                 else
                     own_sort(plan, keys, o1, plan.bitsN, N, E, p, bad, stream);
             };
-            rc = own_zero(plan, p, kHeader, stream);
+            rc = own_zero(plan, p, plan.off_tbl, stream);
             if (rc) return rc;
             if (rank) {
                 int32_t *src32 = reinterpret_cast<int32_t *>(p + align_up(plan.bytes, 256));
                 int32_t *tgt32 = reinterpret_cast<int32_t *>(p + align_up(plan.bytes, 256) + remap_arr_bytes(E));
                 const int vec_ids = (((uintptr_t)edge_index | (uintptr_t)(edge_index + E)) & 15) == 0;
-                hipLaunchKernelGGL(gi_remap_count_kernel, dim3(gi_chunk_grid(plan.n_chunks)), dim3(kRemapTpb), 0, stream, edge_index,
+                auto remap_count = ride ? gi_remap_count_kernel<true> : gi_remap_count_kernel<false>;
+                hipLaunchKernelGGL(remap_count, dim3(gi_chunk_grid(plan.n_chunks)), dim3(kRemapTpb), 0, stream, edge_index,
                                    edge_index + E, E, N, rank, vec_ids, src32, tgt32, plan.chunk, plan.n_chunks,
-                                   own_tbl(plan, p), own_range(plan, p), bad);
+                                   own_tbl(plan, p), own_range(plan, p), bad, tot_s);
                 first_sort(KeysCoo32{src32, tgt32, label, rows, rows ? cy->rows_stride : 0,
                                      (!label || ((uintptr_t)label & 3) == 0) ? 1 : 0});
             } else {
-                own_count(plan, k1, E, p, bad, stream);
+                if (ride)
+                    own_count<KeysCoo, true>(plan, k1, E, p, bad, stream);
+                else
+                    own_count(plan, k1, E, p, bad, stream);
                 first_sort(k1);
             }
             const KeysCsr k2{o->src};
             const OutSrc o2{o->spos, o->spos_inv, o->rowptr_s};
-            rc = own_zero(plan, p, 0, stream);
-            if (rc) return rc;
-            own_count(plan, k2, E, p, bad, stream);
-            own_sort(plan, k2, o2, 0, N, E, p, bad, stream);
+            if (ride) {
+                const int64_t n16 = ((int64_t)(plan.T + 1) * 4 + 15) / 16;
+                hipLaunchKernelGGL(gi_zero_kernel, dim3(stream_grid(n16)), dim3(kTpb), 0, stream,
+                                   reinterpret_cast<uint4 *>(own_tbl(plan, p)), n16, over);
+                own_count(plan, k2, E, p, bad, stream, over);
+                own_sort(plan, k2, o2, 0, N, E, p, bad, stream, over, part_s);
+            } else {
+                rc = own_zero(plan, p, 0, stream);
+                if (rc) return rc;
+                own_count(plan, k2, E, p, bad, stream);
+                own_sort(plan, k2, o2, 0, N, E, p, bad, stream);
+            }
         } else {
             rc = library_build(edge_index, o, p, bad, N, E, rank, stream);
             if (rc) return rc;
@@ -1300,8 +1532,12 @@
 struct OutNode {
     static constexpr uint32_t kValMask = 0xffffffffu;
     static constexpr bool kRows = false;
+    static constexpr bool kCanEmit = false;
     int32_t *perm, *rank;
-    __device__ __forceinline__ void ranked(uint32_t k, uint32_t val, uint32_t) const {
+    __device__ __forceinline__ bool emits() const { return false; }
+    __device__ __forceinline__ uint32_t source(uint32_t) const { return 0u; }
+    __device__ __forceinline__ void emit_one(uint32_t, uint32_t) const {}
+    __device__ __forceinline__ void ranked(uint32_t k, uint32_t val, uint32_t, bool) const {
         perm[k] = (int32_t)val;
         rank[val] = (int32_t)k;
     }
diff --git a/gnn_tracking_amd/edge_classifier.py b/gnn_tracking_amd/edge_classifier.py
--- a/gnn_tracking_amd/edge_classifier.py
+++ b/gnn_tracking_amd/edge_classifier.py
@@ -59,7 +59,8 @@
                                  carry_label=y if isinstance(y, Tensor) and self.training else None,
                                  carry_rows=edge_attr if bf16 and edge_attr.shape[1] == 4 else None,
                                  order_by=None if col is None else (x, col, batch if isinstance(batch, Tensor) else None,
-                                                                    _n_events(data)))
+                                                                    _n_events(data)),
+                                 renumbered=locality.loaded_order(data) is not None)
         E = gi.n_edges
         nperm = gi.node_perm
 
diff --git a/gnn_tracking_amd/ops.py b/gnn_tracking_amd/ops.py
--- a/gnn_tracking_amd/ops.py
+++ b/gnn_tracking_amd/ops.py
@@ -157,6 +157,8 @@
 _VALIDATE = bool(os.environ.get("GNNTRK_VALIDATE"))
 _GI_FLAGS = int(os.environ.get("GNNTRK_GI_FLAGS", "0"))
 CARRY = os.environ.get("GNNTRK_GI_CARRY", "1") != "0"
+GI_RIDE_BIT = 16
+RIDE = os.environ.get("GNNTRK_GI_RIDE", "1") != "0"
 
 
 def node_order(x: Tensor, col: int, batch: Optional[Tensor] = None, n_events: int = 0):
@@ -190,7 +192,7 @@
 def graph_index(edge_index: Tensor, n_nodes: int, *, cache: bool = True,
                 validate: Optional[bool] = None, flags: Optional[int] = None,
                 carry_label: Optional[Tensor] = None, carry_rows: Optional[Tensor] = None,
-                order_by: Optional[tuple] = None) -> GraphIndex:
+                order_by: Optional[tuple] = None, renumbered: bool = False) -> GraphIndex:
     if edge_index.dim() != 2 or edge_index.shape[0] != 2:
         raise ValueError(f"edge_index must be [2,E], got {tuple(edge_index.shape)}")
     if edge_index.dtype != torch.int64:
@@ -231,9 +233,12 @@
         rows_csr = ops_bf16.empty_rows(E, 4, dev)
         cy.edge_rows, cy.rows_csr_bf16 = _p(rows), _p(rows_csr)
         cy.rows_stride, cy.out_stride = int(rows.stride(0)), int(rows_csr.stride(0))
-    ws = _ws(lib.gnntrk_graph_index_workspace_bytes_carry(n_nodes, E, int(rows is not None) | (2 if gi.node_rank is not None else 0)), ei)
-    _capi.check(lib.gnntrk_graph_index_build_carry(_p(ei), C.byref(d), C.byref(cy), _p(ws), ws.numel(),
-                                                   _GI_FLAGS if flags is None else int(flags), _stream(ei)), lib)
+    if flags is None:
+        flags = _GI_FLAGS | (GI_RIDE_BIT if RIDE and (order_by is not None or renumbered) else 0)
+    flags = int(flags)
+    ws = _ws(lib.gnntrk_graph_index_workspace_bytes_carry(
+        n_nodes, E, int(rows is not None) | (2 if gi.node_rank is not None else 0) | (4 if flags & GI_RIDE_BIT else 0)), ei)
+    _capi.check(lib.gnntrk_graph_index_build_carry(_p(ei), C.byref(d), C.byref(cy), _p(ws), ws.numel(), flags, _stream(ei)), lib)
     if lab is not None:
         gi._label_csr = (id(carry_label), carry_label._version, weakref.ref(carry_label), lab_csr)
     if rows is not None:
```

Result: no change. 3.048 billion, median of 6 (+0.8%).
